# Dylan-H-Wang/skin-sm3

Measured on AMD Instinct MI355X. Metric: SM3 pretrain images/sec (paired 224x224), higher is better.
Workload: dtype bf16

## Files before the change

### include/sm3_hip.h

```cpp
#ifndef SM3_HIP_H
#define SM3_HIP_H

#include <stdint.h>

#ifdef __cplusplus
extern "C" {
#endif

#define SM3_F32 0
#define SM3_BF16 1
#define SM3_F16 2

#define SM3_EINVAL (-1)
#define SM3_EALIGN (-2)
#define SM3_EDTYPE (-3)

#define SM3_MAX_TAPS 9

int sm3_abi_version(void);

typedef struct sm3_conv_desc {
    int32_t dtype;
    int32_t N, Hi, Wi, Ci;
    int32_t Ho, Wo, Co;
    int32_t sy, sx;
    int32_t ntaps;
    int32_t dy[SM3_MAX_TAPS], dx[SM3_MAX_TAPS], wtap[SM3_MAX_TAPS];
    int32_t w_row_stride;
    int32_t Hout, Wout;
    int32_t osy, osx, ooy, oox;
} sm3_conv_desc;

int sm3_conv_partial_rows(const sm3_conv_desc* d);

int sm3_conv_gather_gemm(const sm3_conv_desc* d, const void* x, const void* w, void* y,
                         const void* addend, float* stat_partials, void* stream);

typedef struct sm3_bn_bwd_fuse {
    const uint8_t* relu_mask;
    const void* x;
    const float* mean;
    const float* invstd;
    float* partials;
    int32_t partial_row_offset;
    int32_t views;
    int32_t partial_row_offset_view1;
    int32_t addend_sp_h, addend_sp_w;
} sm3_bn_bwd_fuse;
int sm3_conv_dgrad_bnfuse(const sm3_conv_desc* d, const void* dy_in, const void* w_dgrad, void* dz_out,
                          const void* addend, const sm3_bn_bwd_fuse* fuse, void* stream);

typedef struct sm3_conv_seg {
    const void* x1;
    const void* w1;
    int32_t Ci1;
    int64_t w_view_stride;
    int64_t w1_view_stride;
    const float* col_bias;
    int32_t views;
} sm3_conv_seg;
int sm3_conv_dgrad_seg_bnfuse(const sm3_conv_desc* d, const void* x0, const void* w0, const sm3_conv_seg* seg,
                              void* dz_out, const void* addend, const sm3_bn_bwd_fuse* fuse, void* stream);
int sm3_conv_gather_gemm_seg(const sm3_conv_desc* d, const void* x0, const void* w0, const sm3_conv_seg* seg, void* y,
                             const void* addend, void* stream);
int sm3_conv_seg_act(const sm3_conv_desc* d, const void* x0, const void* w0, const sm3_conv_seg* seg, int relu, void* y,
                     uint8_t* relu_mask, void* stream);

int sm3_conv_bn_act_eval(const sm3_conv_desc* d, const void* x, const void* w, const float* scale,
                         const float* shift, const void* residual, int relu, void* y, void* stream);
int sm3_conv_bn_act_fused(const sm3_conv_desc* d, const void* x, const void* w, const float* scale, const float* shift,
                          const void* residual, int relu, void* y, uint8_t* relu_mask, int views, void* stream);
int sm3_conv_bn_eval(const sm3_conv_desc* d, const void* x, const void* w, const float* gamma, const float* beta,
                     const float* running_mean, const float* running_var, float eps, const void* residual, int relu,
                     void* y, void* stream);

int sm3_conv_wgrad(const sm3_conv_desc* d, const void* x, const void* dy, float* dw, void* stream);
int sm3_conv_wgrad_cat(const sm3_conv_desc* d, const void* x, const void* dy, float* dw, const void* dy1, int Co1,
                       float* dw1, int views, int64_t dw_view_stride, int64_t dw1_view_stride, void* stream);
int sm3_conv_wgrad_slabs(const sm3_conv_desc* d, const void* x, const void* dy, float* slabs, int slab_capacity, int views,
                         int* slabs_used, void* stream);
int sm3_slab_reduce(const float* slabs, int nslabs, int64_t n, float* out, int accumulate, void* stream);
int sm3_conv_wgrad_det(const sm3_conv_desc* d, const void* x, const void* dy, float* dw, float* slabs, int slab_capacity,
                       void* stream);

#define SM3_BN_REDUCE_GROUPS 64
int sm3_bn_reduce_groups(int rows);
int sm3_bn_stats_reduce(const float* partials, int rows, int C, double* sums, double* workspace, int views,
                        void* stream);
int sm3_bn_finalize(const double* sums, int groups , int views,
                    double count , int C, const float* gamma, const float* beta,
                    float eps, float momentum, float* running_mean, float* running_var,
                    int64_t* num_batches_tracked , float* scale, float* shift, float* save_mean,
                    float* save_invstd , void* stream);
int sm3_bn_eval_scale_shift(const float* gamma, const float* beta, const float* running_mean,
                            const float* running_var, float eps, int C, float* scale, float* shift,
                            void* stream);
int sm3_bn_act(int dtype, const void* x, const float* scale, const float* shift, const void* residual,
               int relu, int out_f32, void* y, uint8_t* relu_mask, int64_t rows, int C, int views, void* stream);
int sm3_bn_act_colsum_rows(int64_t rows, int C, int dtype);
int sm3_bn_act_colsum(int dtype, const void* x, const float* scale, const float* shift, const void* residual, int relu,
                      void* y, uint8_t* relu_mask, float* colsum_partials, int64_t rows, int C, int views, void* stream);
int sm3_subsample_colsum_rows(int64_t rows, int C, int dtype);
int sm3_subsample_colsum(int dtype, const void* x, void* y, float* colsum_partials, int N, int H, int W, int C, int stride,
                         int views, void* stream);
int sm3_bn_add_bn_act(int dtype, const void* x, const float* scale, const float* shift, const void* x2,
                      const float* scale2, const float* shift2, int relu, void* y, uint8_t* relu_mask,
                      int64_t rows, int C, int views, void* stream);
int sm3_bn_bwd_partial_rows(int64_t rows, int C);
int sm3_bn_bwd_reduce(int dtype, const void* dy, const void* y, const uint8_t* relu_mask, const void* x,
                      const float* mean, const float* invstd, void* dz, int64_t rows, int C,
                      float* partials , int views, void* stream);
int sm3_bn_bwd_apply(int dtype, const void* dz, const void* x, const float* mean, const float* invstd,
                     const float* gamma, const double* global_sums, double count,
                     const double* local_sums, float* dgamma, float* dbeta, void* dx, int64_t rows,
                     int C, int views, void* stream);

typedef struct sm3_bn_apply_side {
    const void* x;
    const float* mean;
    const float* invstd;
    const float* gamma;
    const double* global_sums;
    const double* local_sums;
    float* dgamma;
    float* dbeta;
    void* dx;
} sm3_bn_apply_side;
int sm3_bn_bwd_apply2(int dtype, const void* dz, double count, const sm3_bn_apply_side* a,
                      const sm3_bn_apply_side* b, int64_t rows, int C, int views, void* stream);

int sm3_linbn_moments(const float* slabs, int nslabs, int64_t n, float* out, const float* colsum_partials, int colsum_rows,
                      double* s_out, int p, int views, void* stream);
int sm3_linbn_fwd_stats(int dtype, const float* G, const void* w_dgrad, const void* w_fwd, const double* s, float* Tm,
                        double* sums_ws, int C, int p, int views, void* stream);
int sm3_linbn_stats(int dtype, const float* P, const void* w_fwd, const float* mean, const float* invstd, const float* gamma,
                    const double* reduce_ws, int groups, double* lsums, float* dgamma, float* dbeta, double count,
                    float* coef, int C, int p, int views, void* stream);
int sm3_linbn_coef(const double* global_sums, double count, const float* gamma, const float* mean, const float* invstd,
                   float* coef, int C, int views, void* stream);
int sm3_linbn_banks(int dtype, const void* w_dgrad, const float* coef, void* wa, void* wbn, float* col_const, int C, int p,
                    int views, void* stream);
int sm3_linbn_fold(const double* sums_ws, int groups, int n, int views, double* out, void* stream);
int sm3_linbn_scale_banks(int dtype, const void* w3, int K3, const float* scale3, const float* shift3, void* out3,
                          const void* wd, int Kd, const float* scaled, const float* shiftd, void* outd, float* bias, int C,
                          int views, void* stream);
int sm3_linbn_post(int dtype, const void* wbn, const void* w_dgrad, void* hn, const float* P, const float* G,
                   const float* Tm, const double* s, const float* coef, float* dw, int C, int p, int views, void* stream);
int sm3_linbn_banks_post(int dtype, const void* w_dgrad, const float* coef, void* wa, float* col_const, void* hn,
                         const float* P, const float* G, const float* Tm, const double* s, float* dw, int C, int p, int views,
                         void* stream);

int sm3_stem_partial_rows(int N, int H, int W);
int sm3_stem_weight_prep(int dtype, const float* w_master, void* w_stem, void* stream);
int sm3_stem_weight_prep_if(int dtype, const float* w_master, void* w_stem, const int* only_if, void* stream);
int sm3_stem_conv_fwd(int dtype, const float* x_nchw, const void* w_stem, void* y, float* stat_partials, int N, int H,
                      int W, void* stream);
#define SM3_STEM_WGRAD_SLABS 768
int sm3_stem_wgrad_bn(int dtype, const float* x_nchw, const void* dz, const void* xo, const float* mean,
                      const float* invstd, const float* gamma, const double* global_sums, double count,
                      const double* local_sums, float* dgamma, float* dbeta, float* dw, float* dw_slabs, int N, int H, int W,
                      int views, void* stream);
int sm3_stem_image_cols(int W);
int sm3_stem_image_prep(int dtype, const float* x_view0, const float* x_view1, void* ximg, int n_per_view, int views, int H,
                        int W, void* stream);
int sm3_stem_conv_fwd16(int dtype, const void* ximg, const void* w_stem, void* y, float* stat_partials, int N, int H, int W,
                        void* stream);
int sm3_stem_wgrad_bn16(int dtype, const void* ximg, const void* dz, const void* xo, const float* mean, const float* invstd,
                        const float* gamma, const double* global_sums, double count, const double* local_sums,
                        float* dgamma, float* dbeta, float* dw, float* dw_slabs, int N, int H, int W, int views,
                        void* stream);
int sm3_stem_dgrad_bn(int dtype, const void* dz, const void* xo, const float* mean, const float* invstd, const float* gamma,
                      const double* global_sums, double count, const float* w_master, float* dx, int N, int H, int W,
                      int views, void* stream);
int sm3_maxpool3x3s2_fwd(int dtype, const void* x, void* y, uint8_t* argmax, int N, int H, int W, int C, void* stream);
int sm3_maxpool3x3s2_bwd(int dtype, const uint8_t* argmax, const void* dy, void* dx, int N, int H, int W, int C,
                         void* stream);
int sm3_bn_relu_maxpool_fwd(int dtype, const void* x, const float* scale, const float* shift, void* y,
                            uint8_t* argmax, int N, int H, int W, int C, int views, void* stream);
int sm3_maxpool_bn_bwd_partial_rows(int N, int H, int W, int views);
int sm3_maxpool_bn_bwd(int dtype, const uint8_t* argmax, const void* dy, const void* x, const float* scale,
                       const float* shift, const float* mean, const float* invstd, void* dz, float* partials,
                       int N, int H, int W, int C, int views, void* stream);
int sm3_avgpool_fwd(int dtype, const void* x, float* feat_f32, void* feat_t, int N, int HW, int C, void* stream);
int sm3_avgpool_bwd(int dtype, const void* dfeat, void* dx, int N, int HW, int C, void* stream);

int sm3_weight_prep(int dtype, const float* w, int Co, int taps, int Ci, void* w_fwd, int ld_fwd,
                    void* w_dgrad, void* stream);
typedef struct sm3_wprep_item {
    const float* w;
    void* w_fwd;
    void* w_dgrad;
    int32_t Co, taps, Ci, ld_fwd;
} sm3_wprep_item;
int sm3_weight_prep_batch(int dtype, const sm3_wprep_item* items_device, int n, void* stream);
int sm3_weights_changed(const float* flat, int64_t n, uint64_t* state, int* changed, void* stream);
int sm3_weight_prep_batch_if(int dtype, const sm3_wprep_item* items_device, int n, const int* only_if, void* stream);
int sm3_cast_from_f32(int dtype, const float* src, void* dst, int64_t n, void* stream);
int sm3_cast_to_f32(int dtype, const void* src, float* dst, int64_t n, void* stream);

int sm3_ntxent_logits(const float* z, int R, int D, float temperature, float* zn, float* inv_norm,
                      float* logits, void* stream);
int sm3_ntxent_logits_bwd(int dtype, const float* dlogits, const float* zn, const float* inv_norm, int R,
                          int D, float temperature, void* dz, void* stream);
int sm3_ce_label0(const float* logits, int R, int Cc, float weight, float* row_terms, float* loss, float* dlogits,
                  void* stream);
int sm3_ntxent_fused(int dtype, const float* z, int R, int D, float temperature, float weight,
                     float* workspace, float* loss, void* dz, void* stream);

int sm3_ntxent_fused_scaled(int dtype, const float* z, int R, int D, float temperature, float weight,
                            const float* dz_scale, float* workspace, float* loss, void* dz, void* stream);

int sm3_ntxent_fused_batch(int dtype, int nterms, const float* const* z, int R, int D, float temperature, const float* weights,
                           const float* dz_scale, float* workspace, float* loss, void* const* dz, void* stream);

int sm3_normalize_rows(const float* z, int R, int D, float* zn, float* inv_norm, void* stream);
int sm3_ntxent_rect(float* S, int Rl, int Rg, int self_offset, float temperature, float weight, const float* dz_scale,
                    float* row_terms , float* loss, void* stream);
int sm3_normalize_rows_bwd(int dtype, const float* dzn_a, const float* dzn_b, const float* zn, const float* inv_norm,
                           int R, int D, void* dz, void* stream);

int sm3_adamw(float* p, const float* g, float* m, float* v, int64_t n, float lr, float beta1, float beta2,
              float eps, float weight_decay, int step, float grad_scale, const int32_t* found_inf,
              void* stream);
int sm3_adamw_dynamic(float* p, const float* g, float* m, float* v, int64_t n, float lr, float beta1, float beta2,
                      float eps, float weight_decay, float grad_scale, const float* loss_scale,
                      const int32_t* steps_taken, const int32_t* found_inf, void* stream);
int sm3_loss_scale_update(float* loss_scale, int32_t* found_inf, int32_t* growth_tracker, int32_t* steps_taken,
                          float growth_factor, float backoff_factor, int growth_interval, void* stream);
int sm3_ema_update(float* target, const float* online, int64_t n, float momentum, void* stream);
int sm3_check_finite(const float* g, int64_t n, int32_t* found_inf, void* stream);

int sm3_aug_resized_crop(const uint8_t* src, int B, int Hs, int Ws, const int32_t* box, const uint8_t* flip, float* out,
                         int H, int W, void* stream);
int sm3_aug_resized_crop_ragged(const uint8_t* arena, int64_t arena_bytes, const int64_t* offset, const int32_t* img_h,
                                const int32_t* img_w, int n_images, const int32_t* index, const int32_t* box,
                                const uint8_t* flip, int B, float* out, int H, int W, void* stream);
int sm3_aug_color_op(float* img, int B, int H, int W, const int32_t* op, const float* factor, float* gray_mean, void* stream);
int sm3_aug_finish(const float* img, int B, int H, int W, const uint8_t* gray, const float* sigma, const float* mean3,
                   const float* std3, float* out, void* stream);

int sm3_token_attention(int dtype, const void* qkv, void* out, int B, int S, int D, int nhead, void* stream);
int sm3_add_layernorm(int dtype, const void* a, const void* b, const float* gamma, const float* beta, float eps,
                      void* out, int64_t rows, int D, void* stream);
int sm3_token_heads(int dtype, const void* x, const float* W, const float* bias, const int* token_of, int l2_norm,
                    float* out, int B, int S, int D, int T, void* stream);

int sm3_mlc_attention_fwd(const float* qkv, float* out, int B, int S, int D, int nhead, float p, uint32_t seed,
                          int label_major, void* stream);
int sm3_mlc_attention_bwd(const float* qkv, const float* dout, float* dqkv, int B, int S, int D, int nhead, float p,
                          uint32_t seed, int label_major, void* stream);
int sm3_mlc_add_ln_fwd(const float* a, const float* b, const float* gamma, const float* beta, float eps, float p,
                       uint32_t seed, float* out, float* stats, int64_t rows, int D, void* stream);
int sm3_mlc_add_ln_bwd(const float* dout, const float* a, const float* b, const float* stats, const float* gamma, float p,
                       uint32_t seed, float* da, float* db, float* dgamma, float* dbeta, int64_t rows, int D, void* stream);
int sm3_mlc_bias_relu_drop_fwd(const float* y, const float* bias, float p, uint32_t seed, float* h, float* hd, int64_t rows,
                               int N, void* stream);
int sm3_mlc_relu_drop_bwd(const float* dhd, const float* h, float p, uint32_t seed, float* dh, float* dbias, int64_t rows,
                          int N, void* stream);
int sm3_mlc_colsum(const float* dy, float* db, int64_t rows, int N, void* stream);
int sm3_mlc_ce(const float* logits, const int64_t* targets, const int* head_offsets, int H, int B, int Tn, float temperature,
               float* loss, float* dlogits, void* stream);
int sm3_mlc_heads_fwd(const float* x, const float* W, const float* bias, const int* token_of, int l2_norm, float* out, int B,
                      int S, int D, int Tn, int label_major, void* stream);
int sm3_mlc_heads_bwd(const float* dlogits, const float* x, const float* W, const int* token_of, int l2_norm, float* dx,
                      float* dW, float* dbias, int B, int S, int D, int Tn, int label_major, void* stream);
int sm3_mlc_kmeans_assign(const float* emb, const float* centroids, int64_t* assign, float* sums, int* counts, int N, int D,
                          int K, void* stream);
int sm3_mlc_kmeans_update(float* centroids, const float* sums, const int* counts, int K, int D, void* stream);

#define SM3_MLC_SLAB_ROWS 256
int sm3_mlc_colsum_det(const float* dy, float* db, float* slabs, int64_t rows, int N, int groups, void* stream);
int sm3_mlc_add_ln_bwd_det(const float* dout, const float* a, const float* b, const float* stats, const float* gamma, float p,
                           uint32_t seed, float* da, float* db, float* dgamma, float* dbeta, float* slabs, int64_t rows, int D,
                           void* stream);
int sm3_mlc_heads_bwd_det(const float* dlogits, const float* x, const float* W, const int* token_of, int l2_norm, float* dx,
                          float* dW, float* dbias, float* work, int B, int S, int D, int Tn, int label_major, void* stream);
int sm3_mlc_kmeans_assign_det(const float* emb, const float* centroids, int64_t* assign, float* sums, int* counts, float* slabs,
                              int N, int D, int K, void* stream);

int sm3_grouped_gemm(int dtype, const void* x, const void* w, void* y, float* stat_partials, int rows, int groups, int K, int N,
                     void* stream);
int sm3_grouped_wgrad_det(int dtype, const void* x, const void* dy, float* dw, float* slabs, int slab_capacity, int rows,
                          int groups, int K, int N, void* stream);

int sm3_gconv_weight_prep(int dtype, const float* master, void* w_fwd, void* w_dgrad, int C, int groups, const int* only_if,
                          void* stream);
int sm3_gconv_fwd(int dtype, const void* x, const void* w_fwd, void* y, float* stat_partials, int N, int H, int W, int C,
                  int groups, int stride, void* stream);
int sm3_gconv_dgrad(int dtype, const void* dy, const void* w_dgrad, void* dx, int N, int H, int W, int C, int groups, int stride,
                    void* stream);
int sm3_gconv_wgrad_slabs(int N, int H, int W, int stride, int slab_capacity);
int sm3_gconv_wgrad_det(int dtype, const void* x, const void* dy, float* dw, float* slabs, int slab_capacity, int N, int H,
                        int W, int C, int groups, int stride, void* stream);

int sm3_p2p_mailbox_bytes(void);
int sm3_p2p_max_elems(void);
int sm3_p2p_max_world(void);
int sm3_p2p_layout(int slot, int src, int block, int64_t* data_first, int64_t* data_bytes, int64_t* flag_off,
                   int* elems_per_block);
int sm3_p2p_alloc(void** ptr, void* ipc_handle_64, int* kind_out);
int sm3_p2p_open(const void* ipc_handle_64, void** ptr);
int sm3_p2p_close(void* ptr);
int sm3_p2p_free(void* ptr);
int sm3_p2p_allreduce_f64(double* buf, int n, void* const* mailboxes, int rank, int world, uint64_t seq, int* err_flag,
                          double timeout_s, void* stream);

int sm3_knn_vote(const float* S, int64_t B, int64_t N, int64_t ld, const int32_t* targets, int L, const int32_t* class_offsets,
                 int k, float temperature, float* scores, int32_t* nbr_idx, float* nbr_sim, void* stream);

int sm3_cam_alpha(int dtype, const void* g, float* alpha, int T, int N, int HW, int C, void* stream);
int sm3_cam_maps(int dtype, const void* a, const float* alpha, float* low, float* maps, int N, int T, int h, int w, int C, int H,
                 int W, void* stream);

int sm3_attr_path(const float* x, const float* base, int base_n, float* out, int N, int64_t E, int k0, int c, int steps,
                  void* stream);
int sm3_attr_noise(const float* x, const float* sigma, float* out, int N, int64_t E, int k0, int c, int stride, uint64_t seed,
                   void* stream);
int sm3_attr_accumulate(const float* g, float* acc, int c, int N, int64_t E, float weight, int squared, void* stream);
int sm3_attr_finish_blocks(int HW);
int sm3_attr_finish(const float* acc, const float* x, const float* base, int base_n, float* attr, float* maps, double* sums,
                    double* partials, int T, int N, int C, int HW, int mode, void* stream);

int sm3_faith_rank_workspace(int rows, int HW);
// ... 16 lines not shown
```

### skin-sm3_amd/csrc/pool.hip

```cpp
#include "common.h"

namespace {

template <typename T>
__device__ __forceinline__ void store_elem(T* p, float v);
template <>
__device__ __forceinline__ void store_elem<float>(float* p, float v) { *p = v; }
template <>
__device__ __forceinline__ void store_elem<bf16_t>(bf16_t* p, float v) { p->v = f32_to_bf16(v); }
template <>
__device__ __forceinline__ void store_elem<f16_t>(f16_t* p, float v) { p->v = f32_to_f16(v); }

struct PixDiv {
    FastDiv cv, w, hw;
};
static PixDiv make_pixdiv(int cv, int w, int h) {
    PixDiv d;
    d.cv = make_fastdiv((uint32_t)cv);
    d.w = make_fastdiv((uint32_t)w);
    d.hw = make_fastdiv((uint32_t)(w * h));
    return d;
}
__device__ __forceinline__ void split_index(uint32_t idx, const PixDiv& d, int& c, uint32_t& pix, int& n, int& y, int& x) {
    pix = fdiv(idx, d.cv);
    c = (int)(idx - pix * d.cv.d);
    n = (int)fdiv(pix, d.hw);
    const uint32_t rem = pix - (uint32_t)n * d.hw.d;
    y = (int)fdiv(rem, d.w);
    x = (int)(rem - (uint32_t)y * d.w.d);
}

template <typename T>
__global__ __launch_bounds__(256) void maxpool_fwd_kernel(const T* __restrict__ x, T* __restrict__ y,
                                                          uint8_t* __restrict__ argmax, int N, int H, int W, int C,
                                                          int Ho, int Wo, uint32_t total, const PixDiv dv) {
    constexpr int E = ElemTraits<T>::kPer16B;
    for (uint32_t idx = blockIdx.x * blockDim.x + threadIdx.x; idx < total; idx += gridDim.x * blockDim.x) {
        int c, n, oy, ox;
        uint32_t pix32;
        split_index(idx, dv, c, pix32, n, oy, ox);
        const int64_t pix = pix32;
        float best[E];
        int arg[E];
#pragma unroll
        for (int e = 0; e < E; ++e) {
            best[e] = -INFINITY;
            arg[e] = -1;
        }
#pragma unroll
        for (int kh = 0; kh < 3; ++kh) {
            const int iy = oy * 2 - 1 + kh;
            if ((unsigned)iy >= (unsigned)H) continue;
#pragma unroll
            for (int kw = 0; kw < 3; ++kw) {
                const int ix = ox * 2 - 1 + kw;
                if ((unsigned)ix >= (unsigned)W) continue;
                float v[E];
                unpack16<T>(*reinterpret_cast<const uint4*>(x + (((int64_t)n * H + iy) * W + ix) * C + (int64_t)c * E), v);
#pragma unroll
                for (int e = 0; e < E; ++e)
                    if (v[e] > best[e] || arg[e] < 0) {
                        best[e] = v[e];
                        arg[e] = kh * 3 + kw;
                    }
            }
        }
        *reinterpret_cast<uint4*>(y + pix * C + (int64_t)c * E) = pack16<T>(best);
        if (argmax) {
            uint8_t* a = argmax + pix * C + (int64_t)c * E;
            if constexpr (E == 8) {
                *reinterpret_cast<uint2*>(a) = make_uint2(
                    (unsigned)arg[0] | ((unsigned)arg[1] << 8) | ((unsigned)arg[2] << 16) | ((unsigned)arg[3] << 24),
                    (unsigned)arg[4] | ((unsigned)arg[5] << 8) | ((unsigned)arg[6] << 16) | ((unsigned)arg[7] << 24));
            } else {
                *reinterpret_cast<unsigned*>(a) =
                    (unsigned)arg[0] | ((unsigned)arg[1] << 8) | ((unsigned)arg[2] << 16) | ((unsigned)arg[3] << 24);
            }
        }
    }
}

template <typename T>
__global__ __launch_bounds__(256) void maxpool_bwd_kernel(const uint8_t* __restrict__ argmax, const T* __restrict__ dy,
                                                          T* __restrict__ dx, int N, int H, int W, int C, int Ho,
                                                          int Wo, uint32_t total, const PixDiv dv) {
    constexpr int E = ElemTraits<T>::kPer16B;
    for (uint32_t idx = blockIdx.x * blockDim.x + threadIdx.x; idx < total; idx += gridDim.x * blockDim.x) {
        int c, n, iy, ix;
        uint32_t pix32;
        split_index(idx, dv, c, pix32, n, iy, ix);
        const int64_t pix = pix32;
        float g[E];
#pragma unroll
        for (int e = 0; e < E; ++e) g[e] = 0.f;
        const int oy_lo = iy / 2, oy_hi = min(Ho - 1, (iy + 1) / 2);
        const int ox_lo = ix / 2, ox_hi = min(Wo - 1, (ix + 1) / 2);
        for (int oy = oy_lo; oy <= oy_hi; ++oy)
            for (int ox = ox_lo; ox <= ox_hi; ++ox) {
                const int self = (iy - (oy * 2 - 1)) * 3 + (ix - (ox * 2 - 1));
                const int64_t o = (((int64_t)n * Ho + oy) * Wo + ox) * C + (int64_t)c * E;
                unsigned a[2];
                if constexpr (E == 8) {
                    const uint2 q = *reinterpret_cast<const uint2*>(argmax + o);
                    a[0] = q.x;
                    a[1] = q.y;
                } else {
                    a[0] = *reinterpret_cast<const unsigned*>(argmax + o);
                    a[1] = 0;
                }
                float d[E];
                unpack16<T>(*reinterpret_cast<const uint4*>(dy + o), d);
#pragma unroll
                for (int e = 0; e < E; ++e)
                    if ((int)((a[e >> 2] >> (8 * (e & 3))) & 0xff) == self) g[e] += d[e];
            }
        *reinterpret_cast<uint4*>(dx + pix * C + (int64_t)c * E) = pack16<T>(g);
    }
}

template <typename T>
__global__ __launch_bounds__(256) void bn_relu_maxpool_fwd_kernel(const T* __restrict__ x, const float* __restrict__ scale,
                                                                  const float* __restrict__ shift, T* __restrict__ y,
                                                                  uint8_t* __restrict__ argmax, int N, int H, int W, int C,
                                                                  int Ho, int Wo, int n_per_view, uint32_t total,
                                                                  const PixDiv dv) {
    constexpr int E = ElemTraits<T>::kPer16B;
    for (uint32_t idx = blockIdx.x * blockDim.x + threadIdx.x; idx < total; idx += gridDim.x * blockDim.x) {
        int c, n, oy, ox;
        uint32_t pix32;
        split_index(idx, dv, c, pix32, n, oy, ox);
        const int64_t pix = pix32;
        const int view = n / n_per_view;
        float sc[E], sh[E], best[E];
        int arg[E];
#pragma unroll
        for (int e = 0; e < E; ++e) {
            sc[e] = scale[view * C + c * E + e];
            sh[e] = shift[view * C + c * E + e];
            best[e] = -INFINITY;
            arg[e] = -1;
        }
#pragma unroll
        for (int kh = 0; kh < 3; ++kh) {
            const int iy = oy * 2 - 1 + kh;
            if ((unsigned)iy >= (unsigned)H) continue;
#pragma unroll
            for (int kw = 0; kw < 3; ++kw) {
                const int ix = ox * 2 - 1 + kw;
                if ((unsigned)ix >= (unsigned)W) continue;
                float v[E];
                unpack16<T>(*reinterpret_cast<const uint4*>(x + (((int64_t)n * H + iy) * W + ix) * C + (int64_t)c * E), v);
#pragma unroll
                for (int e = 0; e < E; ++e) {
                    const float a = ElemTraits<T>::round(fmaxf(v[e] * sc[e] + sh[e], 0.f));
                    if (a > best[e] || arg[e] < 0) {
                        best[e] = a;
                        arg[e] = kh * 3 + kw;
                    }
                }
            }
        }
        *reinterpret_cast<uint4*>(y + pix * C + (int64_t)c * E) = pack16<T>(best);
        if (argmax) {
            uint8_t* a = argmax + pix * C + (int64_t)c * E;
            if constexpr (E == 8) {
                *reinterpret_cast<uint2*>(a) = make_uint2(
                    (unsigned)arg[0] | ((unsigned)arg[1] << 8) | ((unsigned)arg[2] << 16) | ((unsigned)arg[3] << 24),
                    (unsigned)arg[4] | ((unsigned)arg[5] << 8) | ((unsigned)arg[6] << 16) | ((unsigned)arg[7] << 24));
            } else {
                *reinterpret_cast<unsigned*>(a) =
                    (unsigned)arg[0] | ((unsigned)arg[1] << 8) | ((unsigned)arg[2] << 16) | ((unsigned)arg[3] << 24);
            }
        }
    }
}

template <typename T>
__global__ __launch_bounds__(256) void maxpool_bn_bwd_kernel(const uint8_t* __restrict__ argmax, const T* __restrict__ dy,
                                                             const T* __restrict__ x, const float* __restrict__ scale,
                                                             const float* __restrict__ shift,
                                                             const float* __restrict__ mean,
                                                             const float* __restrict__ invstd, T* __restrict__ dz,
                                                             float* __restrict__ partials, int H, int W, int C, int Ho,
                                                             int Wo, int n_per_view, int64_t rows, int tbx, int tby,
                                                             const FastDiv div_hw, const FastDiv div_w) {
    constexpr int E = ElemTraits<T>::kPer16B;
    __shared__ float sred[256 * 2 * 8];
    const int tx = threadIdx.x % tbx, ty = threadIdx.x / tbx;
    const int cv = blockIdx.x * tbx + tx;
    const bool active = (cv * E < C) && (ty < tby);
    const int view = blockIdx.z;
    float s1[E], s2[E];
#pragma unroll
    for (int e = 0; e < E; ++e) s1[e] = s2[e] = 0.f;
    if (active) {
        float sc[E], sh[E], mu[E], is[E];
#pragma unroll
        for (int e = 0; e < E; ++e) {
            sc[e] = scale[view * C + cv * E + e];
            sh[e] = shift[view * C + cv * E + e];
            mu[e] = mean[view * C + cv * E + e];
            is[e] = invstd[view * C + cv * E + e];
        }
        constexpr int U = 2;
        const int64_t rstep = (int64_t)gridDim.y * tby;
        for (int64_t r0 = (int64_t)blockIdx.y * tby + ty; r0 < rows; r0 += U * rstep) {
            uint4 xu[U], du[U][4];
            unsigned au[U][4][2];
            int selfs[U][4];
            int64_t pixs[U];
#pragma unroll
            for (int u = 0; u < U; ++u) {
                const int64_t r = r0 + u * rstep;
                pixs[u] = -1;
                xu[u] = make_uint4(0, 0, 0, 0);
#pragma unroll
                for (int w = 0; w < 4; ++w) selfs[u][w] = -1;
                if (r >= rows) continue;
                const uint32_t nl = fdiv((uint32_t)r, div_hw);
                const uint32_t rem = (uint32_t)r - nl * div_hw.d;
                const int iy = (int)fdiv(rem, div_w), ix = (int)(rem - (uint32_t)iy * div_w.d);
                const int64_t n = (int64_t)view * n_per_view + nl;
                pixs[u] = (int64_t)view * rows + r;
                xu[u] = ldg16<true>(x + pixs[u] * C + (int64_t)cv * E);
                const int oy_lo = iy / 2, oy_hi = min(Ho - 1, (iy + 1) / 2);
                const int ox_lo = ix / 2, ox_hi = min(Wo - 1, (ix + 1) / 2);
#pragma unroll
                for (int w = 0; w < 4; ++w) {
                    const int oy = oy_lo + (w >> 1), ox = ox_lo + (w & 1);
                    if (oy > oy_hi || ox > ox_hi) continue;
                    selfs[u][w] = (iy - (oy * 2 - 1)) * 3 + (ix - (ox * 2 - 1));
                    const int64_t o = ((n * Ho + oy) * Wo + ox) * C + (int64_t)cv * E;
                    if constexpr (E == 8) {
                        const uint2 q = *reinterpret_cast<const uint2*>(argmax + o);
                        au[u][w][0] = q.x;
                        au[u][w][1] = q.y;
                    } else {
                        au[u][w][0] = *reinterpret_cast<const unsigned*>(argmax + o);
                        au[u][w][1] = 0;
                    }
                    du[u][w] = *reinterpret_cast<const uint4*>(dy + o);
                }
            }
#pragma unroll
            for (int u = 0; u < U; ++u) {
                if (pixs[u] < 0) continue;
                float g[E];
#pragma unroll
                for (int e = 0; e < E; ++e) g[e] = 0.f;
#pragma unroll
                for (int w = 0; w < 4; ++w) {
                    if (selfs[u][w] < 0) continue;
                    float d[E];
                    unpack16<T>(du[u][w], d);
#pragma unroll
                    for (int e = 0; e < E; ++e)
                        if ((int)((au[u][w][e >> 2] >> (8 * (e & 3))) & 0xff) == selfs[u][w]) g[e] += d[e];
                }
                float xv[E];
                unpack16<T>(xu[u], xv);
#pragma unroll
                for (int e = 0; e < E; ++e) g[e] = (xv[e] * sc[e] + sh[e] > ElemTraits<T>::kReluBit) ? g[e] : 0.f;
                const uint4 packed = pack16<T>(g);
                stg16<true>(dz + pixs[u] * C + (int64_t)cv * E, packed);
                float gr[E];
                unpack16<T>(packed, gr);
#pragma unroll
                for (int e = 0; e < E; ++e) {
                    s1[e] += gr[e];
                    s2[e] += gr[e] * (xv[e] - mu[e]) * is[e];
                }
            }
        }
    }
    float* mine = sred + threadIdx.x * 2 * E;
#pragma unroll
    for (int e = 0; e < E; ++e) {
        mine[e] = s1[e];
        mine[E + e] = s2[e];
    }
    __syncthreads();
    if (ty == 0 && cv * E < C) {
        for (int j = 1; j < tby; ++j) {
            const float* o = sred + (j * tbx + tx) * 2 * E;
#pragma unroll
            for (int e = 0; e < E; ++e) {
                s1[e] += o[e];
                s2[e] += o[E + e];
            }
        }
        float* pv = partials + (int64_t)view * gridDim.y * 2 * C;
        float* p1 = pv + ((int64_t)blockIdx.y * 2 + 0) * C + (int64_t)cv * E;
        float* p2 = pv + ((int64_t)blockIdx.y * 2 + 1) * C + (int64_t)cv * E;
#pragma unroll
        for (int e = 0; e < E; ++e) {
            p1[e] = s1[e];
            p2[e] = s2[e];
        }
    }
}

template <typename T>
__global__ __launch_bounds__(256) void avgpool_fwd_kernel(const T* __restrict__ x, float* __restrict__ f32,
                                                          T* __restrict__ ft, int N, int HW, int C) {
    constexpr int E = ElemTraits<T>::kPer16B;
    const int cv = C / E;
    const int64_t total = (int64_t)N * cv;
    const int64_t idx = (int64_t)blockIdx.x * blockDim.x + threadIdx.x;
    if (idx >= total) return;
    const int c = (int)(idx % cv);
    const int n = (int)(idx / cv);
    float s[E];
#pragma unroll
    for (int e = 0; e < E; ++e) s[e] = 0.f;
    for (int i = 0; i < HW; ++i) {
        float v[E];
        unpack16<T>(*reinterpret_cast<const uint4*>(x + ((int64_t)n * HW + i) * C + (int64_t)c * E), v);
#pragma unroll
        for (int e = 0; e < E; ++e) s[e] += v[e];
    }
    const float inv = 1.f / (float)HW;
#pragma unroll
    for (int e = 0; e < E; ++e) s[e] *= inv;
    if (f32) {
#pragma unroll
        for (int e = 0; e < E; ++e) f32[(int64_t)n * C + (int64_t)c * E + e] = s[e];
    }
    if (ft) *reinterpret_cast<uint4*>(ft + (int64_t)n * C + (int64_t)c * E) = pack16<T>(s);
}

template <typename T>
__global__ __launch_bounds__(256) void avgpool_bwd_kernel(const T* __restrict__ df, T* __restrict__ dx, int N, int HW,
                                                          int C) {
    constexpr int E = ElemTraits<T>::kPer16B;
    const int cv = C / E;
    const int64_t total = (int64_t)N * HW * cv;
    const float inv = 1.f / (float)HW;
    for (int64_t idx = (int64_t)blockIdx.x * blockDim.x + threadIdx.x; idx < total;
         idx += (int64_t)gridDim.x * blockDim.x) {
        const int c = (int)(idx % cv);
        const int64_t pix = idx / cv;
        const int n = (int)(pix / HW);
        float v[E];
        unpack16<T>(*reinterpret_cast<const uint4*>(df + (int64_t)n * C + (int64_t)c * E), v);
#pragma unroll
        for (int e = 0; e < E; ++e) v[e] *= inv;
        *reinterpret_cast<uint4*>(dx + pix * C + (int64_t)c * E) = pack16<T>(v);
    }
}

template <typename T>
__global__ void weight_prep_kernel(const float* __restrict__ w, int Co, int taps, int Ci, T* __restrict__ wf, int ld,
                                   T* __restrict__ wd) {
    const int64_t nf = wf ? (int64_t)Co * ld : 0;
    const int64_t nd = wd ? (int64_t)Co * taps * Ci : 0;
    const int K = taps * Ci;
    for (int64_t idx = (int64_t)blockIdx.x * blockDim.x + threadIdx.x; idx < nf + nd;
         idx += (int64_t)gridDim.x * blockDim.x) {
        if (idx < nf) {
            const int co = (int)(idx / ld), k = (int)(idx % ld);
            store_elem<T>(wf + idx, k < K ? w[(int64_t)co * K + k] : 0.f);
        } else {
            const int64_t j = idx - nf;
            const int co = (int)(j % Co);
            const int t = (int)((j / Co) % taps);
            const int ci = (int)(j / ((int64_t)Co * taps));
            store_elem<T>(wd + j, w[((int64_t)co * taps + t) * Ci + ci]);
        }
    }
}

template <typename T>
__global__ __launch_bounds__(256) void weight_prep_batch_kernel(const sm3_wprep_item* __restrict__ items,
                                                                const int* __restrict__ only_if) {
    __shared__ float tile[32][33];
    if (only_if && *only_if == 0) return;
    const sm3_wprep_item it = items[blockIdx.y];
    const float* __restrict__ w = it.w;
    T* __restrict__ wf = reinterpret_cast<T*>(it.w_fwd);
    T* __restrict__ wd = reinterpret_cast<T*>(it.w_dgrad);
    const int Co = it.Co, taps = it.taps, Ci = it.Ci, ld = it.ld_fwd, K = taps * Ci;
    const bool vec = sizeof(T) == 2 && ld == K && (K & 3) == 0 && (Co & 1) == 0 && ((uintptr_t)w & 15) == 0 &&
                     ((uintptr_t)wf & 7) == 0 && ((uintptr_t)wd & 3) == 0;
    if (wf && vec) {
        const int64_t nq = (int64_t)Co * K / 4;
        const float4* __restrict__ w4 = reinterpret_cast<const float4*>(w);
        uint2* __restrict__ o2 = reinterpret_cast<uint2*>(wf);
        for (int64_t q = (int64_t)blockIdx.x * blockDim.x + threadIdx.x; q < nq; q += (int64_t)gridDim.x * blockDim.x) {
            const float4 v = w4[q];
            uint2 o;
            if constexpr (sizeof(T) == 2) {
                o.x = pack2<T>(v.x, v.y);
                o.y = pack2<T>(v.z, v.w);
            }
            o2[q] = o;
        }
    } else if (wf) {
        const int64_t nf = (int64_t)Co * ld;
        for (int64_t idx = (int64_t)blockIdx.x * blockDim.x + threadIdx.x; idx < nf; idx += (int64_t)gridDim.x * blockDim.x) {
            const int co = (int)(idx / ld), k = (int)(idx % ld);
            store_elem<T>(wf + idx, k < K ? w[(int64_t)co * K + k] : 0.f);
        }
    }
    if (wd && vec) {
        __shared__ float tile2[64][33];
        const int tco = (Co + 63) / 64, tci = (Ci + 31) / 32;
        const int ntiles = taps * tco * tci;
        const int tx = threadIdx.x & 31, ty = threadIdx.x >> 5;
        for (int tl = blockIdx.x; tl < ntiles; tl += gridDim.x) {
            const int t = tl / (tco * tci), r = tl - t * tco * tci;
            const int co0 = (r / tci) * 64, ci0 = (r % tci) * 32;
#pragma unroll
            for (int j = 0; j < 8; ++j) {
                const int co = co0 + ty + 8 * j, ci = ci0 + tx;
                tile2[ty + 8 * j][tx] = (co < Co && ci < Ci) ? w[((int64_t)co * taps + t) * Ci + ci] : 0.f;
            }
            __syncthreads();
#pragma unroll
            for (int j = 0; j < 4; ++j) {
                const int ci = ci0 + ty + 8 * j, co = co0 + 2 * tx;
                if constexpr (sizeof(T) == 2) {
                    if (ci < Ci && co < Co)
                        *reinterpret_cast<uint32_t*>(wd + ((int64_t)ci * taps + t) * Co + co) =
                            pack2<T>(tile2[2 * tx][ty + 8 * j], tile2[2 * tx + 1][ty + 8 * j]);
                }
            }
            __syncthreads();
        }
    } else if (wd) {
        const int tco = (Co + 31) / 32, tci = (Ci + 31) / 32;
        const int ntiles = taps * tco * tci;
        const int tx = threadIdx.x & 31, ty = threadIdx.x >> 5;
        for (int tl = blockIdx.x; tl < ntiles; tl += gridDim.x) {
            const int t = tl / (tco * tci), r = tl - t * tco * tci;
            const int co0 = (r / tci) * 32, ci0 = (r % tci) * 32;
#pragma unroll
            for (int j = 0; j < 4; ++j) {
                const int co = co0 + ty + 8 * j, ci = ci0 + tx;
                tile[ty + 8 * j][tx] = (co < Co && ci < Ci) ? w[((int64_t)co * taps + t) * Ci + ci] : 0.f;
            }
            __syncthreads();
#pragma unroll
            for (int j = 0; j < 4; ++j) {
                const int ci = ci0 + ty + 8 * j, co = co0 + tx;
                if (ci < Ci && co < Co) store_elem<T>(wd + ((int64_t)ci * taps + t) * Co + co, tile[tx][ty + 8 * j]);
            }
            __syncthreads();
        }
    }
}

template <typename T>
__global__ void cast_from_f32_kernel(const float* __restrict__ s, T* __restrict__ d, int64_t n) {
    for (int64_t i = (int64_t)blockIdx.x * blockDim.x + threadIdx.x; i < n; i += (int64_t)gridDim.x * blockDim.x)
        store_elem<T>(d + i, s[i]);
}
template <typename T>
__global__ void cast_to_f32_kernel(const T* __restrict__ s, float* __restrict__ d, int64_t n) {
    for (int64_t i = (int64_t)blockIdx.x * blockDim.x + threadIdx.x; i < n; i += (int64_t)gridDim.x * blockDim.x)
        d[i] = ElemTraits<T>::load(s + i);
}

inline unsigned grid_for(int64_t total, int per_block = 256, int64_t cap = 8192) {
    int64_t g = (total + per_block - 1) / per_block;
    if (g > cap) g = cap;
    if (g < 1) g = 1;
    return (unsigned)g;
}

}

#define DISPATCH_T(dtype, CALL_F32, CALL_BF16, CALL_F16)  \
    if ((dtype) == SM3_F32) { CALL_F32; }       \
    else if ((dtype) == SM3_BF16) { CALL_BF16; } \
    else if ((dtype) == SM3_F16) { CALL_F16; } \
    else return SM3_EDTYPE;

extern "C" int sm3_maxpool3x3s2_fwd(int dtype, const void* x, void* y, uint8_t* argmax, int N, int H, int W, int C,
                                    void* stream) {
    if (!x || !y || N <= 0 || H <= 0 || W <= 0 || C <= 0) return SM3_EINVAL;
    const int E = dtype == SM3_F32 ? 4 : 8;
    if (C % E) return SM3_EALIGN;
    const int Ho = (H + 2 - 3) / 2 + 1, Wo = (W + 2 - 3) / 2 + 1;
    const int64_t total = (int64_t)N * Ho * Wo * (C / E);
    if (total >= 0x7fffffffLL) return SM3_EINVAL;
    const unsigned g = grid_for(total, 256, 1 << 20);
    hipStream_t st = (hipStream_t)stream;
    const PixDiv dv = make_pixdiv(C / E, Wo, Ho);
    DISPATCH_T(dtype,
               hipLaunchKernelGGL(maxpool_fwd_kernel<float>, dim3(g), dim3(256), 0, st, (const float*)x, (float*)y, argmax, N, H, W, C, Ho, Wo, (uint32_t)total, dv),
               hipLaunchKernelGGL(maxpool_fwd_kernel<bf16_t>, dim3(g), dim3(256), 0, st, (const bf16_t*)x, (bf16_t*)y, argmax, N, H, W, C, Ho, Wo, (uint32_t)total, dv),
               hipLaunchKernelGGL(maxpool_fwd_kernel<f16_t>, dim3(g), dim3(256), 0, st, (const f16_t*)x, (f16_t*)y, argmax, N, H, W, C, Ho, Wo, (uint32_t)total, dv));
    SM3_CHECK_LAUNCH();
    return 0;
}

extern "C" int sm3_maxpool3x3s2_bwd(int dtype, const uint8_t* argmax, const void* dy, void* dx, int N, int H, int W,
                                    int C, void* stream) {
    if (!argmax || !dy || !dx || N <= 0 || H <= 0 || W <= 0 || C <= 0) return SM3_EINVAL;
    const int E = dtype == SM3_F32 ? 4 : 8;
    if (C % E) return SM3_EALIGN;
    const int Ho = (H + 2 - 3) / 2 + 1, Wo = (W + 2 - 3) / 2 + 1;
    const int64_t total = (int64_t)N * H * W * (C / E);
    if (total >= 0x7fffffffLL) return SM3_EINVAL;
    const unsigned g = grid_for(total, 256, 1 << 20);
    hipStream_t st = (hipStream_t)stream;
    const PixDiv dv = make_pixdiv(C / E, W, H);
    DISPATCH_T(dtype,
               hipLaunchKernelGGL(maxpool_bwd_kernel<float>, dim3(g), dim3(256), 0, st, argmax, (const float*)dy, (float*)dx, N, H, W, C, Ho, Wo, (uint32_t)total, dv),
               hipLaunchKernelGGL(maxpool_bwd_kernel<bf16_t>, dim3(g), dim3(256), 0, st, argmax, (const bf16_t*)dy, (bf16_t*)dx, N, H, W, C, Ho, Wo, (uint32_t)total, dv),
               hipLaunchKernelGGL(maxpool_bwd_kernel<f16_t>, dim3(g), dim3(256), 0, st, argmax, (const f16_t*)dy, (f16_t*)dx, N, H, W, C, Ho, Wo, (uint32_t)total, dv));
    SM3_CHECK_LAUNCH();
    return 0;
}

extern "C" int sm3_bn_relu_maxpool_fwd(int dtype, const void* x, const float* scale, const float* shift, void* y,
                                       uint8_t* argmax, int N, int H, int W, int C, int views, void* stream) {
    if (!x || !scale || !shift || !y || N <= 0 || H <= 0 || W <= 0 || C <= 0 || views < 1 || N % views) return SM3_EINVAL;
    if (!SM3_DTYPE_OK(dtype)) return SM3_EDTYPE;
    const int E = dtype == SM3_F32 ? 4 : 8;
    if (C % E) return SM3_EALIGN;
    const int Ho = (H + 2 - 3) / 2 + 1, Wo = (W + 2 - 3) / 2 + 1;
    const int64_t total = (int64_t)N * Ho * Wo * (C / E);
    if (total >= 0x7fffffffLL) return SM3_EINVAL;
    const unsigned g = grid_for(total, 256, 1 << 20);
    hipStream_t st = (hipStream_t)stream;
    const PixDiv dv = make_pixdiv(C / E, Wo, Ho);
    DISPATCH_T(dtype,
               hipLaunchKernelGGL(bn_relu_maxpool_fwd_kernel<float>, dim3(g), dim3(256), 0, st, (const float*)x, scale, shift, (float*)y, argmax, N, H, W, C, Ho, Wo, N / views, (uint32_t)total, dv),
               hipLaunchKernelGGL(bn_relu_maxpool_fwd_kernel<bf16_t>, dim3(g), dim3(256), 0, st, (const bf16_t*)x, scale, shift, (bf16_t*)y, argmax, N, H, W, C, Ho, Wo, N / views, (uint32_t)total, dv),
               hipLaunchKernelGGL(bn_relu_maxpool_fwd_kernel<f16_t>, dim3(g), dim3(256), 0, st, (const f16_t*)x, scale, shift, (f16_t*)y, argmax, N, H, W, C, Ho, Wo, N / views, (uint32_t)total, dv));
    SM3_CHECK_LAUNCH();
    return 0;
}

extern "C" int sm3_maxpool_bn_bwd_partial_rows(int N, int H, int W, int views) {
    if (N <= 0 || H <= 0 || W <= 0 || views < 1 || N % views) return SM3_EINVAL;
    int64_t gy = ((int64_t)(N / views) * H * W + 63) / 64;
    return (int)(gy > 1024 ? 1024 : gy);
}

extern "C" int sm3_maxpool_bn_bwd(int dtype, const uint8_t* argmax, const void* dy, const void* x, const float* scale,
                                  const float* shift, const float* mean, const float* invstd, void* dz,
                                  float* partials, int N, int H, int W, int C, int views, void* stream) {
    if (!argmax || !dy || !x || !scale || !shift || !mean || !invstd || !dz || !partials) return SM3_EINVAL;
    if (N <= 0 || H <= 0 || W <= 0 || C <= 0 || views < 1 || N % views) return SM3_EINVAL;
    if (!SM3_DTYPE_OK(dtype)) return SM3_EDTYPE;
    const int E = dtype == SM3_F32 ? 4 : 8;
    if (C % E || C / E > 256) return SM3_EALIGN;
    const int Ho = (H + 2 - 3) / 2 + 1, Wo = (W + 2 - 3) / 2 + 1;
    const int64_t rows = (int64_t)(N / views) * H * W;
    if (rows * views >= 0x7fffffffLL) return SM3_EINVAL;
    const int cvecs = C / E;
    int tbx = 1;
    while (tbx < cvecs && tbx < 256) tbx <<= 1;
    const int tby = 256 / tbx;
    const int gx = (cvecs + tbx - 1) / tbx;
    const int gy = sm3_maxpool_bn_bwd_partial_rows(N, H, W, views);
    hipStream_t st = (hipStream_t)stream;
    const FastDiv dhw = make_fastdiv((uint32_t)(H * W)), dw = make_fastdiv((uint32_t)W);
    dim3 grid(gx, gy, views);
    DISPATCH_T(dtype,
               hipLaunchKernelGGL(maxpool_bn_bwd_kernel<float>, grid, dim3(256), 0, st, argmax, (const float*)dy, (const float*)x, scale, shift, mean, invstd, (float*)dz, partials, H, W, C, Ho, Wo, N / views, rows, tbx, tby, dhw, dw),
               hipLaunchKernelGGL(maxpool_bn_bwd_kernel<bf16_t>, grid, dim3(256), 0, st, argmax, (const bf16_t*)dy, (const bf16_t*)x, scale, shift, mean, invstd, (bf16_t*)dz, partials, H, W, C, Ho, Wo, N / views, rows, tbx, tby, dhw, dw),
               hipLaunchKernelGGL(maxpool_bn_bwd_kernel<f16_t>, grid, dim3(256), 0, st, argmax, (const f16_t*)dy, (const f16_t*)x, scale, shift, mean, invstd, (f16_t*)dz, partials, H, W, C, Ho, Wo, N / views, rows, tbx, tby, dhw, dw));
    SM3_CHECK_LAUNCH();
    return 0;
}

extern "C" int sm3_avgpool_fwd(int dtype, const void* x, float* feat_f32, void* feat_t, int N, int HW, int C,
                               void* stream) {
    if (!x || N <= 0 || HW <= 0 || C <= 0 || (!feat_f32 && !feat_t)) return SM3_EINVAL;
    const int E = dtype == SM3_F32 ? 4 : 8;
    if (C % E) return SM3_EALIGN;
    const int64_t total = (int64_t)N * (C / E);
    const unsigned g = (unsigned)((total + 255) / 256);
    hipStream_t st = (hipStream_t)stream;
    DISPATCH_T(dtype,
               hipLaunchKernelGGL(avgpool_fwd_kernel<float>, dim3(g), dim3(256), 0, st, (const float*)x, feat_f32, (float*)feat_t, N, HW, C),
               hipLaunchKernelGGL(avgpool_fwd_kernel<bf16_t>, dim3(g), dim3(256), 0, st, (const bf16_t*)x, feat_f32, (bf16_t*)feat_t, N, HW, C),
               hipLaunchKernelGGL(avgpool_fwd_kernel<f16_t>, dim3(g), dim3(256), 0, st, (const f16_t*)x, feat_f32, (f16_t*)feat_t, N, HW, C));
    SM3_CHECK_LAUNCH();
    return 0;
}

extern "C" int sm3_avgpool_bwd(int dtype, const void* dfeat, void* dx, int N, int HW, int C, void* stream) {
    if (!dfeat || !dx || N <= 0 || HW <= 0 || C <= 0) return SM3_EINVAL;
    const int E = dtype == SM3_F32 ? 4 : 8;
    if (C % E) return SM3_EALIGN;
    const unsigned g = grid_for((int64_t)N * HW * (C / E));
    hipStream_t st = (hipStream_t)stream;
    DISPATCH_T(dtype,
               hipLaunchKernelGGL(avgpool_bwd_kernel<float>, dim3(g), dim3(256), 0, st, (const float*)dfeat, (float*)dx, N, HW, C),
               hipLaunchKernelGGL(avgpool_bwd_kernel<bf16_t>, dim3(g), dim3(256), 0, st, (const bf16_t*)dfeat, (bf16_t*)dx, N, HW, C),
               hipLaunchKernelGGL(avgpool_bwd_kernel<f16_t>, dim3(g), dim3(256), 0, st, (const f16_t*)dfeat, (f16_t*)dx, N, HW, C));
    SM3_CHECK_LAUNCH();
    return 0;
}

extern "C" int sm3_weight_prep(int dtype, const float* w, int Co, int taps, int Ci, void* w_fwd, int ld_fwd,
                               void* w_dgrad, void* stream) {
    if (!w || Co <= 0 || taps <= 0 || Ci <= 0 || (!w_fwd && !w_dgrad)) return SM3_EINVAL;
    if (w_fwd && ld_fwd < taps * Ci) return SM3_EINVAL;
    const int64_t total = (w_fwd ? (int64_t)Co * ld_fwd : 0) + (w_dgrad ? (int64_t)Co * taps * Ci : 0);
    const unsigned g = grid_for(total);
    hipStream_t st = (hipStream_t)stream;
    DISPATCH_T(dtype,
               hipLaunchKernelGGL(weight_prep_kernel<float>, dim3(g), dim3(256), 0, st, w, Co, taps, Ci, (float*)w_fwd, ld_fwd, (float*)w_dgrad),
               hipLaunchKernelGGL(weight_prep_kernel<bf16_t>, dim3(g), dim3(256), 0, st, w, Co, taps, Ci, (bf16_t*)w_fwd, ld_fwd, (bf16_t*)w_dgrad),
               hipLaunchKernelGGL(weight_prep_kernel<f16_t>, dim3(g), dim3(256), 0, st, w, Co, taps, Ci, (f16_t*)w_fwd, ld_fwd, (f16_t*)w_dgrad));
    SM3_CHECK_LAUNCH();
    return 0;
}

extern "C" int sm3_weight_prep_batch_if(int dtype, const sm3_wprep_item* items_device, int n, const int* only_if,
                                        void* stream) {
    if (!items_device || n <= 0 || n > 65535) return SM3_EINVAL;
    static const int kWprepGx = getenv("SM3_WPREP_GX") ? atoi(getenv("SM3_WPREP_GX")) : 384;
    hipStream_t st = (hipStream_t)stream;
    DISPATCH_T(dtype,
               hipLaunchKernelGGL(weight_prep_batch_kernel<float>, dim3(kWprepGx, n), dim3(256), 0, st, items_device, only_if),
               hipLaunchKernelGGL(weight_prep_batch_kernel<bf16_t>, dim3(kWprepGx, n), dim3(256), 0, st, items_device, only_if),
               hipLaunchKernelGGL(weight_prep_batch_kernel<f16_t>, dim3(kWprepGx, n), dim3(256), 0, st, items_device, only_if));
    SM3_CHECK_LAUNCH();
    return 0;
}

extern "C" int sm3_weight_prep_batch(int dtype, const sm3_wprep_item* items_device, int n, void* stream) {
    return sm3_weight_prep_batch_if(dtype, items_device, n, nullptr, stream);
}

namespace {

__global__ __launch_bounds__(256) void weights_hash_kernel(const uint32_t* __restrict__ w, int64_t n,
                                                           unsigned long long* __restrict__ acc) {
    unsigned long long h = 0;
    const int64_t stride = (int64_t)gridDim.x * blockDim.x;
    for (int64_t i = (int64_t)blockIdx.x * blockDim.x + threadIdx.x; i < n; i += stride)
        h += ((unsigned long long)w[i] + 0x9E3779B97F4A7C15ull) * (unsigned long long)(2 * i + 1);
#pragma unroll
    for (int o = 32; o > 0; o >>= 1) h += __shfl_xor(h, o, 64);
    __shared__ unsigned long long part[4];
    if ((threadIdx.x & 63) == 0) part[threadIdx.x >> 6] = h;
    __syncthreads();
    if (threadIdx.x == 0) atomicAdd(acc, part[0] + part[1] + part[2] + part[3]);
}

__global__ void weights_changed_kernel(unsigned long long* __restrict__ state, int* __restrict__ changed) {
    *changed = state[0] != state[1];
    state[1] = state[0];
    state[0] = 0;
}

}

extern "C" int sm3_weights_changed(const float* flat, int64_t n, uint64_t* state, int* changed, void* stream) {
    if (!flat || !state || !changed || n <= 0) return SM3_EINVAL;
    hipStream_t st = (hipStream_t)stream;
    hipLaunchKernelGGL(weights_hash_kernel, dim3(1024), dim3(256), 0, st, reinterpret_cast<const uint32_t*>(flat), n,
                       reinterpret_cast<unsigned long long*>(state));
    SM3_CHECK_LAUNCH();
    hipLaunchKernelGGL(weights_changed_kernel, dim3(1), dim3(1), 0, st, reinterpret_cast<unsigned long long*>(state), changed);
    SM3_CHECK_LAUNCH();
    return 0;
}

extern "C" int sm3_cast_from_f32(int dtype, const float* src, void* dst, int64_t n, void* stream) {
    if (!src || !dst || n <= 0) return SM3_EINVAL;
    const unsigned g = grid_for(n);
    hipStream_t st = (hipStream_t)stream;
    DISPATCH_T(dtype,
               hipLaunchKernelGGL(cast_from_f32_kernel<float>, dim3(g), dim3(256), 0, st, src, (float*)dst, n),
               hipLaunchKernelGGL(cast_from_f32_kernel<bf16_t>, dim3(g), dim3(256), 0, st, src, (bf16_t*)dst, n),
               hipLaunchKernelGGL(cast_from_f32_kernel<f16_t>, dim3(g), dim3(256), 0, st, src, (f16_t*)dst, n));
    SM3_CHECK_LAUNCH();
    return 0;
}

extern "C" int sm3_cast_to_f32(int dtype, const void* src, float* dst, int64_t n, void* stream) {
    if (!src || !dst || n <= 0) return SM3_EINVAL;
    const unsigned g = grid_for(n);
    hipStream_t st = (hipStream_t)stream;
    DISPATCH_T(dtype,
               hipLaunchKernelGGL(cast_to_f32_kernel<float>, dim3(g), dim3(256), 0, st, (const float*)src, dst, n),
               hipLaunchKernelGGL(cast_to_f32_kernel<bf16_t>, dim3(g), dim3(256), 0, st, (const bf16_t*)src, dst, n),
               hipLaunchKernelGGL(cast_to_f32_kernel<f16_t>, dim3(g), dim3(256), 0, st, (const f16_t*)src, dst, n));
    SM3_CHECK_LAUNCH();
    return 0;
}
```

### skin-sm3_amd/csrc/stem.hip

```cpp
#include <atomic>

#include "conv_common.h"

namespace {

constexpr int PW = 264;
constexpr int NG = 21;
constexpr int KS = 11;
constexpr int KPAD = KS * 16;
constexpr int OUT_PITCH = 144;

struct StemTile {
    int n, oy, x0;
};
__device__ __forceinline__ StemTile decode_tile(long t, int xblocks, int Ho) {
    StemTile s;
    const int xb = (int)(t % xblocks);
    const long r = t / xblocks;
    s.oy = (int)(r % Ho);
    s.n = (int)(r / Ho);
    s.x0 = xb * 128;
    return s;
}

// ... 277 lines not shown
constexpr int PATCH16 = PDMA * 1024;

template <typename T>
__global__ __launch_bounds__(256) void stem_image_prep_kernel(const float* __restrict__ x0, const float* __restrict__ x1,
                                                              uint4* __restrict__ out, int n_per_view, int H, int W, int Wp8,
                                                              long chunks) {
    const long i = (long)blockIdx.x * 256 + threadIdx.x;
    if (i >= chunks) return;
    const int j = (int)(i % Wp8);
    const long r = i / Wp8;
    const long rows_img = 3L * H;
    const int n = (int)(r / rows_img);
    const long rr = r - (long)n * rows_img;
    const float* src = (n < n_per_view ? x0 + (long)n * rows_img * W : x1 + (long)(n - n_per_view) * rows_img * W) + rr * W;
    float v[8];
    const int q0 = 8 * j - 4;
    if ((W & 3) == 0 && q0 >= 0 && q0 + 8 < W && (((uintptr_t)src) & 15) == 0) {
        const float4 a = *reinterpret_cast<const float4*>(src + q0), b = *reinterpret_cast<const float4*>(src + q0 + 4);
        v[0] = a.y; v[1] = a.z; v[2] = a.w; v[3] = b.x; v[4] = b.y; v[5] = b.z; v[6] = b.w; v[7] = src[q0 + 8];
    } else {
#pragma unroll
        for (int e = 0; e < 8; ++e) {
            const int q = 8 * j + e - 3;
            v[e] = (unsigned)q < (unsigned)W ? src[q] : 0.f;
        }
    }
    out[i] = make_uint4(pack2<T>(v[0], v[1]), pack2<T>(v[2], v[3]), pack2<T>(v[4], v[5]), pack2<T>(v[6], v[7]));
}

struct TileDiv {
    FastDiv xb, ho;
};
__device__ __forceinline__ StemTile decode_tile32(uint32_t t, const TileDiv& d) {
    StemTile s;
    const uint32_t r = fdiv(t, d.xb), xb = t - r * d.xb.d;
    const uint32_t n = fdiv(r, d.ho);
    s.oy = (int)(r - n * d.ho.d);
    s.n = (int)n;
    s.x0 = (int)xb * 128;
    return s;
}

__device__ __forceinline__ void patch_dma(__amdgpu_buffer_rsrc_t rs, uint32_t lds_patch, const StemTile& t, int H, int Wp,
                                          int wave, int lane) {
    for (int k = wave; k < PDMA; k += 4) {
        const int idx = k * 64 + lane;
        const int g = idx / PCH, j = idx - g * PCH;
        const int kh = g / 3, c = g - 3 * kh;
        const int iy = 2 * t.oy - 3 + kh, q = 2 * t.x0 + 8 * j;
        const bool ok = g < NG && (unsigned)iy < (unsigned)H && q < Wp;
        const uint32_t off = ok ? (uint32_t)((((long)t.n * 3 + c) * H + iy) * Wp + q) * 2u : sm3conv::kOOB;
        sm3conv::dma16(rs, lds_patch + (uint32_t)k * 1024u, off, 0u);
    }
}

constexpr int FWD16_LDS = 2 * PATCH16 + 128 * OUT_PITCH + 4 * 64 * 2 * 4 + 64 * (KPAD + 8) * 2;

template <typename T>
__global__ __launch_bounds__(256, 2) void stem_fwd16_kernel(const char* __restrict__ ximg, uint32_t ximg_bytes,
                                                          const uint4* __restrict__ w, T* __restrict__ y,
                                                          float* __restrict__ partials, int H, int Wp, int Ho, int Wo,
                                                          const TileDiv td, uint32_t tiles) {
    extern __shared__ __attribute__((aligned(16))) char smem16[];
    char* sPatch = smem16;
    char* sOut = smem16 + 2 * PATCH16;
    float(*sStat)[64][2] = reinterpret_cast<float(*)[64][2]>(sOut + 128 * OUT_PITCH);
    constexpr int WP = KPAD + 8;
    uint16_t* sW = reinterpret_cast<uint16_t*>(sOut + 128 * OUT_PITCH + 4 * 64 * 2 * 4);
    const int tid = threadIdx.x, lane = tid & 63, wave = __builtin_amdgcn_readfirstlane(tid >> 6);
    const int col = lane & 31, h = lane >> 5;
    for (int i = tid; i < 64 * (KPAD / 8); i += 256) {
        const int co = i / (KPAD / 8), c8 = i - co * (KPAD / 8);
        *reinterpret_cast<uint4*>(&sW[co * WP + c8 * 8]) = w[i];
    }
    const uint16_t* wlane = &sW[col * WP + 8 * h];
    const __amdgpu_buffer_rsrc_t rs = __builtin_amdgcn_make_buffer_rsrc((void*)ximg, 0, ximg_bytes, 0x00020000);
    const uint32_t lds_patch = (uint32_t)(uintptr_t)((__attribute__((address_space(3))) char*)sPatch);

    int buf = 0;
    if (blockIdx.x < tiles) patch_dma(rs, lds_patch, decode_tile32(blockIdx.x, td), H, Wp, wave, lane);
    sm3conv::dma_drain();
    for (uint32_t t = blockIdx.x; t < tiles; t += gridDim.x, buf ^= 1) {
        const StemTile tl = decode_tile32(t, td);
        const uint32_t tn = t + gridDim.x;
        __syncthreads();
        if (tn < tiles)
            patch_dma(rs, lds_patch + (uint32_t)((buf ^ 1) * PATCH16), decode_tile32(tn, td), H, Wp, wave, lane);
        f32x16 acc[2];
#pragma unroll
        for (int nb = 0; nb < 2; ++nb)
#pragma unroll
            for (int r = 0; r < 16; ++r) acc[nb][r] = 0.f;
        const int px = 32 * wave + col;
        const char* prow = sPatch + buf * PATCH16 + 4 * px;
#pragma unroll
        for (int ks = 0; ks < KS; ++ks) {
            const int g = 2 * ks + h;
            uint4 a = make_uint4(0, 0, 0, 0);
            if (g < NG) {
                const uint32_t* src = reinterpret_cast<const uint32_t*>(prow + g * PROW16);
                a = make_uint4(src[0], src[1], src[2], src[3]);
            }
#pragma unroll
            for (int nb = 0; nb < 2; ++nb)
                sm3conv::mma_frag<T>(a, *reinterpret_cast<const uint4*>(wlane + nb * 32 * WP + ks * 16), acc[nb]);
        }
#pragma unroll
        for (int nb = 0; nb < 2; ++nb) {
            float s1 = 0.f, s2 = 0.f;
#pragma unroll
            for (int r = 0; r < 16; ++r) {
                const int row = 32 * wave + (r & 3) + 8 * (r >> 2) + 4 * h;
                const uint16_t b = (uint16_t)pack2<T>(acc[nb][r], 0.f);
                *reinterpret_cast<uint16_t*>(sOut + row * OUT_PITCH + (nb * 32 + col) * 2) = b;
                if (tl.x0 + row < Wo) {
                    const float v = ElemTraits<T>::round(acc[nb][r]);
                    s1 += v;
                    s2 += v * v;
                }
            }
            s1 += __shfl_xor(s1, 32, 64);
            s2 += __shfl_xor(s2, 32, 64);
            if (lane < 32) {
                sStat[wave][nb * 32 + lane][0] = s1;
                sStat[wave][nb * 32 + lane][1] = s2;
            }
        }
        sm3conv::dma_drain();
        __syncthreads();
        if (partials && tid < 128) {
            const int c = tid & 63, st = tid >> 6;
            partials[((long)t * 2 + st) * 64 + c] = (sStat[0][c][st] + sStat[1][c][st]) + (sStat[2][c][st] + sStat[3][c][st]);
        }
        {
            const int ch = tid & 7, r0 = tid >> 3;
            const long pix0 = ((long)tl.n * Ho + tl.oy) * Wo + tl.x0;
#pragma unroll
            for (int k = 0; k < 4; ++k) {
                const int row = r0 + 32 * k;
                if (tl.x0 + row < Wo)
                    stg16<true>(y + (pix0 + row) * 64 + ch * 8,
                                *reinterpret_cast<const uint4*>(sOut + row * OUT_PITCH + ch * 16));
            }
        }
    }
}

struct StemWgrad16Params {
    StemWgradParams q;
    const char* ximg;
    uint32_t ximg_bytes;
    int Wp;
    TileDiv td;
};

template <typename T>
__global__ __launch_bounds__(256, 3) void stem_wgrad16_kernel(const StemWgrad16Params pp) {
    const StemWgradParams& p = pp.q;
    __shared__ __attribute__((aligned(16))) char sPatch[2 * PATCH16];
    __shared__ __attribute__((aligned(16))) char sD[128 * 128];
    __shared__ __attribute__((aligned(16))) float sCoef[3][64];
    const int tid = threadIdx.x, lane = tid & 63, wave = __builtin_amdgcn_readfirstlane(tid >> 6);
    const int cb = wave & 1, kb0 = 3 * (wave >> 1);

    if (blockIdx.x == 0 && tid < 64 && p.lsums) {
        float db = 0.f, dg = 0.f;
        for (int v = 0; v < p.views; ++v) {
            db += (float)p.lsums[v * 128 + tid];
            dg += (float)p.lsums[v * 128 + 64 + tid];
        }
        if (p.dbeta) atomicAdd(&p.dbeta[tid], db);
        if (p.dgamma) atomicAdd(&p.dgamma[tid], dg);
    }

    f32x16 acc[3];
#pragma unroll
    for (int j = 0; j < 3; ++j)
#pragma unroll
        for (int r = 0; r < 16; ++r) acc[j][r] = 0.f;

    const int ch = tid & 7, r0 = tid >> 3;
    int cur_view = -1;
    const int g16 = lane >> 4, ii = lane & 15, qq = ii >> 2, pq = ii & 3, hh = g16 >> 1;
    const uint32_t ra_off = (uint32_t)(8 * hh + qq) * 128u + ((((uint32_t)(cb * 32 + 16 * (g16 & 1) + 4 * pq)) * 2u) ^ swz128(qq));
    const int bn = lane & 31, bh = lane >> 5;
    const __amdgpu_buffer_rsrc_t rs = __builtin_amdgcn_make_buffer_rsrc((void*)pp.ximg, 0, pp.ximg_bytes, 0x00020000);
    const uint32_t lds_patch = (uint32_t)(uintptr_t)((__attribute__((address_space(3))) char*)sPatch);
    uint32_t b_off[3], b_sel[3];
#pragma unroll
    for (int j = 0; j < 3; ++j) {
        const int k = 32 * (kb0 + j) + bn, g = k >> 3, kw = k & 7;
        b_off[j] = g < NG ? (uint32_t)(g * PROW16 + 4 * (8 * bh + (kw >> 1))) : 0xffffffffu;
        b_sel[j] = (kw & 1) ? 0x07060302u : 0x05040100u;
    }

    auto stage_dxo = [&](const StemTile& tl) {
        const int view = tl.n / p.n_per_view;
        if (view != cur_view) {
            cur_view = view;
            if (tid < 64) {
                const int c = tid;
                const float is = p.invstd[view * 64 + c];
                const float g = p.gamma ? p.gamma[c] : 1.f;
                const float k0c = g * is;
                const float k1c = (float)(p.gsums[view * 128 + c] * p.inv_count);
                const float qc = k0c * is * (float)(p.gsums[view * 128 + 64 + c] * p.inv_count);
                sCoef[0][c] = k0c;
                sCoef[1][c] = qc;
                sCoef[2][c] = qc * p.mean[view * 64 + c] - k0c * k1c;
            }
            __syncthreads();
        }
        float cA[8], cB[8], cC[8];
#pragma unroll
        for (int e = 0; e < 8; e += 4) {
            *reinterpret_cast<float4*>(cA + e) = *reinterpret_cast<const float4*>(&sCoef[0][ch * 8 + e]);
            *reinterpret_cast<float4*>(cB + e) = *reinterpret_cast<const float4*>(&sCoef[1][ch * 8 + e]);
            *reinterpret_cast<float4*>(cC + e) = *reinterpret_cast<const float4*>(&sCoef[2][ch * 8 + e]);
        }
        const long pix0 = ((long)tl.n * p.Ho + tl.oy) * p.Wo + tl.x0;
#pragma unroll
        for (int kb = 0; kb < 4; kb += 2) {
            uint4 gu[2], xu[2];
#pragma unroll
            for (int k = 0; k < 2; ++k) {
                const int row = r0 + 32 * (kb + k);
                const bool ok = tl.x0 + row < p.Wo;
                gu[k] = ok ? ldg16<true>(p.dz + ((pix0 + row) * 64 + ch * 8) * 2) : make_uint4(0, 0, 0, 0);
                xu[k] = ok ? ldg16<true>(p.xo + ((pix0 + row) * 64 + ch * 8) * 2) : make_uint4(0, 0, 0, 0);
            }
#pragma unroll
            for (int k = 0; k < 2; ++k) {
                const int row = r0 + 32 * (kb + k);
                uint4 out = make_uint4(0, 0, 0, 0);
                if (tl.x0 + row < p.Wo) {
                    float g[8], xv[8];
                    unpack16<T>(gu[k], g);
                    unpack16<T>(xu[k], xv);
#pragma unroll
                    for (int e = 0; e < 8; ++e) g[e] = cA[e] * g[e] - cB[e] * xv[e] + cC[e];
                    out = pack16<T>(g);
                }
                *reinterpret_cast<uint4*>(sD + row * 128 + (((uint32_t)ch * 16u) ^ swz128(row))) = out;
            }
        }
    };

    int buf = 0;
    const uint32_t ntiles = (uint32_t)p.tiles;
    if (blockIdx.x < ntiles) {
        const StemTile t0 = decode_tile32(blockIdx.x, pp.td);
        patch_dma(rs, lds_patch, t0, p.H, pp.Wp, wave, lane);
        stage_dxo(t0);
    }
    sm3conv::dma_drain();
    for (uint32_t t = blockIdx.x; t < ntiles; t += gridDim.x, buf ^= 1) {
        const uint32_t tn = t + gridDim.x;
        __syncthreads();
        StemTile nx = {0, 0, 0};
        if (tn < ntiles) {
            nx = decode_tile32(tn, pp.td);
            patch_dma(rs, lds_patch + (uint32_t)((buf ^ 1) * PATCH16), nx, p.H, pp.Wp, wave, lane);
        }
        const char* patch = sPatch + buf * PATCH16;
#pragma unroll
        for (int s = 0; s < 8; ++s) {
            const char* a0 = sD + ra_off + s * 16 * 128;
            const s16x4 lo = __builtin_amdgcn_ds_read_tr16_b64_v4i16((__attribute__((address_space(3))) s16x4*)(a0));
            const s16x4 hi = __builtin_amdgcn_ds_read_tr16_b64_v4i16((__attribute__((address_space(3))) s16x4*)(a0 + 4 * 128));
            const uint2 l2 = __builtin_bit_cast(uint2, lo), h2 = __builtin_bit_cast(uint2, hi);
            const uint4 fa = make_uint4(l2.x, l2.y, h2.x, h2.y);
#pragma unroll
            for (int j = 0; j < 3; ++j) {
                uint4 fb = make_uint4(0, 0, 0, 0);
                if (b_off[j] != 0xffffffffu) {
                    const uint32_t* d = reinterpret_cast<const uint32_t*>(patch + b_off[j] + s * 64);
                    fb = make_uint4(__builtin_amdgcn_perm(d[1], d[0], b_sel[j]), __builtin_amdgcn_perm(d[3], d[2], b_sel[j]),
                                    __builtin_amdgcn_perm(d[5], d[4], b_sel[j]), __builtin_amdgcn_perm(d[7], d[6], b_sel[j]));
                }
                sm3conv::mma_frag<T>(fa, fb, acc[j]);
            }
        }
        __syncthreads();
        if (tn < ntiles) stage_dxo(nx);
        sm3conv::dma_drain();
    }

    const int frow = lane & 31, fh = lane >> 5;
#pragma unroll
    for (int j = 0; j < 3; ++j) {
        const int k = 32 * (kb0 + j) + frow;
        const int g = k >> 3, kw = k & 7;
        if (g >= NG || kw >= 7) continue;
        const int kh = g / 3, c = g - 3 * kh;
        const int kcol = (kh * 7 + kw) * 3 + c;
#pragma unroll
        for (int r = 0; r < 16; ++r) {
            const int co = cb * 32 + (r & 3) + 8 * (r >> 2) + 4 * fh;
            if (p.dw_slabs) p.dw_slabs[(long)blockIdx.x * (64 * 147) + co * 147 + kcol] = acc[j][r];
            else atomicAdd(p.dw + co * 147 + kcol, acc[j][r]);
        }
    }
}

template <typename T>
__global__ void stem_weight_prep_kernel(const float* __restrict__ w, T* __restrict__ out, const int* __restrict__ only_if) {
    const int i = blockIdx.x * blockDim.x + threadIdx.x;
    if (i >= 64 * KPAD || (only_if && *only_if == 0)) return;
    const int co = i / KPAD, k = i - co * KPAD;
    const int g = k >> 3, kw = k & 7;
    float v = 0.f;
    if (g < NG && kw < 7) {
        const int kh = g / 3, c = g - 3 * kh;
        v = w[co * 147 + (kh * 7 + kw) * 3 + c];
    }
    out[i].v = (uint16_t)pack2<T>(v, 0.f);
}


constexpr int WPF = 172;

__global__ __launch_bounds__(256, 2) void stem_fwd_f32_kernel(const float* __restrict__ x, const float* __restrict__ w,
                                                              float* __restrict__ y, float* __restrict__ partials, int N,
                                                              int H, int W, int Ho, int Wo, int xblocks, long tiles) {
    __shared__ __attribute__((aligned(16))) float patch[NG * PW];
    __shared__ float sStat[4][64][2];
    __shared__ __attribute__((aligned(16))) float sW[64 * WPF];
    const int tid = threadIdx.x, lane = tid & 63, wave = tid >> 6;
    const int col = lane & 31, h = lane >> 5;
    for (int i = tid; i < 64 * (NG * 8 / 4); i += 256) {
        const int co = i / (NG * 2), c4 = i - co * (NG * 2);
        *reinterpret_cast<float4*>(&sW[co * WPF + c4 * 4]) = *reinterpret_cast<const float4*>(w + (long)co * KPAD + c4 * 4);
    }
    const float* wlane = &sW[col * WPF + 4 * h];

    PatchRegs pre;
    if ((long)blockIdx.x < tiles) {
        load_patch(pre, x, decode_tile(blockIdx.x, xblocks, Ho), H, W);
        store_patch(patch, pre);
    }
    __syncthreads();
    for (long t = blockIdx.x; t < tiles; t += gridDim.x) {
        const StemTile tl = decode_tile(t, xblocks, Ho);
        const long tn = t + gridDim.x;
        if (tn < tiles) load_patch(pre, x, decode_tile(tn, xblocks, Ho), H, W);
        f32x16 acc[2];
#pragma unroll
        for (int nb = 0; nb < 2; ++nb)
#pragma unroll
            for (int r = 0; r < 16; ++r) acc[nb][r] = 0.f;
        const int px = 32 * wave + col;
#pragma unroll
        for (int g = 0; g < NG; ++g) {
            const float2* src = reinterpret_cast<const float2*>(patch + g * PW + 2 * px + 4 * h);
            const float2 v0 = src[0], v1 = src[1];
            const uint4 a = make_uint4(__float_as_uint(v0.x), __float_as_uint(v0.y), __float_as_uint(v1.x), __float_as_uint(v1.y));
#pragma unroll
            for (int nb = 0; nb < 2; ++nb)
                sm3conv::mma_frag<float>(a, *reinterpret_cast<const uint4*>(wlane + nb * 32 * WPF + g * 8), acc[nb]);
        }
        const long pix0 = ((long)tl.n * Ho + tl.oy) * Wo + tl.x0;
#pragma unroll
        for (int nb = 0; nb < 2; ++nb) {
            float s1 = 0.f, s2 = 0.f;
#pragma unroll
            for (int r = 0; r < 16; ++r) {
                const int row = 32 * wave + (r & 3) + 8 * (r >> 2) + 4 * h;
                if (tl.x0 + row < Wo) {
                    const float v = acc[nb][r];
                    y[(pix0 + row) * 64 + nb * 32 + col] = v;
                    s1 += v;
                    s2 += v * v;
                }
            }
            s1 += __shfl_xor(s1, 32, 64);
            s2 += __shfl_xor(s2, 32, 64);
            if (lane < 32) {
                sStat[wave][nb * 32 + lane][0] = s1;
                sStat[wave][nb * 32 + lane][1] = s2;
            }
        }
        __syncthreads();
        if (partials && tid < 128) {
            const int c = tid & 63, st = tid >> 6;
            partials[(t * 2 + st) * 64 + c] = (sStat[0][c][st] + sStat[1][c][st]) + (sStat[2][c][st] + sStat[3][c][st]);
        }
        if (tn < tiles) store_patch(patch, pre);
        __syncthreads();
    }
}

__global__ __launch_bounds__(256, 2) void stem_wgrad_f32_kernel(const StemWgradParams p) {
    __shared__ __attribute__((aligned(16))) float patch[NG * PW];
    __shared__ __attribute__((aligned(16))) float sD[128 * 64];
    __shared__ __attribute__((aligned(16))) float sCoef[3][64];
    const int tid = threadIdx.x, lane = tid & 63, wave = tid >> 6;
// ... 313 lines not shown
    tiles = (long)N * Ho * xblocks;
    if ((long)N * 3 * H * W >= 0x7fffffffL || (long)N * Ho * Wo >= 0x7fffffffL / 64) return SM3_EINVAL;
    return 0;
}

}

extern "C" int sm3_stem_partial_rows(int N, int H, int W) {
    int Ho, Wo, xb;
    long tiles;
    if (stem_geometry(N, H, W, Ho, Wo, xb, tiles)) return SM3_EINVAL;
    return tiles > 0x7fffffffL ? SM3_EINVAL : (int)tiles;
}

extern "C" int sm3_stem_weight_prep_if(int dtype, const float* w_master, void* w_stem, const int* only_if, void* stream) {
    if (!w_master || !w_stem) return SM3_EINVAL;
    if (dtype == SM3_BF16)
        hipLaunchKernelGGL(stem_weight_prep_kernel<bf16_t>, dim3((64 * KPAD + 255) / 256), dim3(256), 0, (hipStream_t)stream,
                           w_master, (bf16_t*)w_stem, only_if);
    else if (dtype == SM3_F16)
        hipLaunchKernelGGL(stem_weight_prep_kernel<f16_t>, dim3((64 * KPAD + 255) / 256), dim3(256), 0, (hipStream_t)stream,
                           w_master, (f16_t*)w_stem, only_if);
    else if (dtype == SM3_F32)
        hipLaunchKernelGGL(stem_weight_prep_f32_kernel, dim3((64 * KPAD + 255) / 256), dim3(256), 0, (hipStream_t)stream,
                           w_master, (float*)w_stem, only_if);
    else
        return SM3_EDTYPE;
    SM3_CHECK_LAUNCH();
    return 0;
}

extern "C" int sm3_stem_weight_prep(int dtype, const float* w_master, void* w_stem, void* stream) {
    return sm3_stem_weight_prep_if(dtype, w_master, w_stem, nullptr, stream);
}

extern "C" int sm3_stem_conv_fwd(int dtype, const float* x_nchw, const void* w_stem, void* y, float* stat_partials, int N,
                                 int H, int W, void* stream) {
    if (!x_nchw || !w_stem || !y) return SM3_EINVAL;
    if (dtype != SM3_BF16 && dtype != SM3_F16 && dtype != SM3_F32) return SM3_EDTYPE;
    int Ho, Wo, xb;
    long tiles;
    if (int rc = stem_geometry(N, H, W, Ho, Wo, xb, tiles)) return rc;
    if (dtype == SM3_F32) {
        const unsigned gridf = (unsigned)(tiles < 512 ? tiles : 512);
        hipLaunchKernelGGL(stem_fwd_f32_kernel, dim3(gridf), dim3(256), 0, (hipStream_t)stream, x_nchw, (const float*)w_stem,
                           (float*)y, stat_partials, N, H, W, Ho, Wo, xb, tiles);
        SM3_CHECK_LAUNCH();
        return 0;
    }
    const unsigned grid = (unsigned)(tiles < 768 ? tiles : 768);
    if (dtype == SM3_BF16)
        hipLaunchKernelGGL(stem_fwd_kernel<bf16_t>, dim3(grid), dim3(256), 0, (hipStream_t)stream, x_nchw,
                           (const uint4*)w_stem, (bf16_t*)y, stat_partials, N, H, W, Ho, Wo, xb, tiles);
    else
        hipLaunchKernelGGL(stem_fwd_kernel<f16_t>, dim3(grid), dim3(256), 0, (hipStream_t)stream, x_nchw,
                           (const uint4*)w_stem, (f16_t*)y, stat_partials, N, H, W, Ho, Wo, xb, tiles);
    SM3_CHECK_LAUNCH();
    return 0;
}

extern "C" int sm3_stem_wgrad_bn(int dtype, const float* x_nchw, const void* dz, const void* xo, const float* mean,
                                 const float* invstd, const float* gamma, const double* global_sums, double count,
                                 const double* local_sums, float* dgamma, float* dbeta, float* dw, float* dw_slabs,
                                 int N, int H, int W, int views, void* stream) {
    if (!x_nchw || !dz || !xo || !mean || !invstd || !global_sums || !dw || count <= 0 || views < 1 || N % views)
        return SM3_EINVAL;
    if (dw_slabs && (((uintptr_t)dw_slabs | (uintptr_t)dw) & 15)) return SM3_EALIGN;
    if (dtype != SM3_BF16 && dtype != SM3_F16 && dtype != SM3_F32) return SM3_EDTYPE;
    StemWgradParams p;
    if (int rc = stem_geometry(N, H, W, p.Ho, p.Wo, p.xblocks, p.tiles)) return rc;
    p.x = x_nchw; p.dz = (const char*)dz; p.xo = (const char*)xo;
    p.mean = mean; p.invstd = invstd; p.gamma = gamma; p.gsums = global_sums; p.lsums = local_sums;
    p.dgamma = dgamma; p.dbeta = dbeta; p.dw = dw; p.dw_slabs = dw_slabs; p.inv_count = 1.0 / count;
    p.N = N; p.H = H; p.W = W; p.n_per_view = N / views; p.views = views;
    if (dtype == SM3_F32) {
        const unsigned gridf = (unsigned)(p.tiles < 512 ? p.tiles : 512);
        hipLaunchKernelGGL(stem_wgrad_f32_kernel, dim3(gridf), dim3(256), 0, (hipStream_t)stream, p);
        SM3_CHECK_LAUNCH();
        return dw_slabs ? sm3_slab_reduce(dw_slabs, (int)gridf, 64 * 147, dw, 1, stream) : 0;
    }
    const unsigned grid = (unsigned)(p.tiles < SM3_STEM_WGRAD_SLABS ? p.tiles : SM3_STEM_WGRAD_SLABS);
    if (dtype == SM3_BF16)
        hipLaunchKernelGGL(stem_wgrad_kernel<bf16_t>, dim3(grid), dim3(256), 0, (hipStream_t)stream, p);
    else
        hipLaunchKernelGGL(stem_wgrad_kernel<f16_t>, dim3(grid), dim3(256), 0, (hipStream_t)stream, p);
    SM3_CHECK_LAUNCH();
    return dw_slabs ? sm3_slab_reduce(dw_slabs, (int)grid, 64 * 147, dw, 1, stream) : 0;
}

extern "C" int sm3_stem_image_cols(int W) { return W > 0 ? (W + 6 + 7) / 8 * 8 : SM3_EINVAL; }

extern "C" int sm3_stem_image_prep(int dtype, const float* x_view0, const float* x_view1, void* ximg, int n_per_view,
                                   int views, int H, int W, void* stream) {
    if (!x_view0 || !ximg || n_per_view <= 0 || H <= 0 || W <= 0 || views < 1 || views > 2 || (views == 2 && !x_view1))
        return SM3_EINVAL;
    if (dtype != SM3_BF16 && dtype != SM3_F16) return SM3_EDTYPE;
    if ((uintptr_t)ximg & 15) return SM3_EALIGN;
    const int Wp = sm3_stem_image_cols(W);
    const long chunks = (long)n_per_view * views * 3 * H * (Wp / 8);
    if (chunks * 16 >= 0xC0000000L) return SM3_EINVAL;
    const long blocks = (chunks + 255) / 256;
    if (dtype == SM3_BF16)
        hipLaunchKernelGGL(stem_image_prep_kernel<bf16_t>, dim3((unsigned)blocks), dim3(256), 0, (hipStream_t)stream, x_view0,
                           x_view1, (uint4*)ximg, n_per_view, H, W, Wp / 8, chunks);
    else
        hipLaunchKernelGGL(stem_image_prep_kernel<f16_t>, dim3((unsigned)blocks), dim3(256), 0, (hipStream_t)stream, x_view0,
                           x_view1, (uint4*)ximg, n_per_view, H, W, Wp / 8, chunks);
    SM3_CHECK_LAUNCH();
    return 0;
}

template <typename K>
static int stem16_allow_lds(K kern, int bytes) {
    static std::atomic<int> done[32];
    int dev = 0;
    if (hipGetDevice(&dev) != hipSuccess || dev < 0 || dev > 31) dev = 0;
    if (!done[dev].load(std::memory_order_acquire)) {
        hipError_t e = hipFuncSetAttribute(reinterpret_cast<const void*>(kern), hipFuncAttributeMaxDynamicSharedMemorySize, bytes);
        if (e != hipSuccess) return (int)e;
        done[dev].store(1, std::memory_order_release);
    }
    return 0;
}

extern "C" int sm3_stem_conv_fwd16(int dtype, const void* ximg, const void* w_stem, void* y, float* stat_partials, int N,
                                   int H, int W, void* stream) {
    if (!ximg || !w_stem || !y) return SM3_EINVAL;
    if (dtype != SM3_BF16 && dtype != SM3_F16) return SM3_EDTYPE;
    int Ho, Wo, xb;
    long tiles;
    if (int rc = stem_geometry(N, H, W, Ho, Wo, xb, tiles)) return rc;
    const int Wp = sm3_stem_image_cols(W);
    const long bytes = (long)N * 3 * H * Wp * 2;
    if (bytes >= 0xC0000000L) return SM3_EINVAL;
    if (tiles > 0x7fffffffL) return SM3_EINVAL;
    const TileDiv td{make_fastdiv((uint32_t)xb), make_fastdiv((uint32_t)Ho)};
    const unsigned grid = (unsigned)(tiles < 512 ? tiles : 512);
    if (dtype == SM3_BF16) {
        if (int rc = stem16_allow_lds(stem_fwd16_kernel<bf16_t>, FWD16_LDS)) return rc;
        hipLaunchKernelGGL(stem_fwd16_kernel<bf16_t>, dim3(grid), dim3(256), FWD16_LDS, (hipStream_t)stream, (const char*)ximg,
                           (uint32_t)bytes, (const uint4*)w_stem, (bf16_t*)y, stat_partials, H, Wp, Ho, Wo, td, (uint32_t)tiles);
    } else {
        if (int rc = stem16_allow_lds(stem_fwd16_kernel<f16_t>, FWD16_LDS)) return rc;
        hipLaunchKernelGGL(stem_fwd16_kernel<f16_t>, dim3(grid), dim3(256), FWD16_LDS, (hipStream_t)stream, (const char*)ximg,
                           (uint32_t)bytes, (const uint4*)w_stem, (f16_t*)y, stat_partials, H, Wp, Ho, Wo, td, (uint32_t)tiles);
    }
    SM3_CHECK_LAUNCH();
    return 0;
}

extern "C" int sm3_stem_wgrad_bn16(int dtype, const void* ximg, const void* dz, const void* xo, const float* mean,
                                   const float* invstd, const float* gamma, const double* global_sums, double count,
                                   const double* local_sums, float* dgamma, float* dbeta, float* dw, float* dw_slabs,
                                   int N, int H, int W, int views, void* stream) {
    if (!ximg || !dz || !xo || !mean || !invstd || !global_sums || !dw || count <= 0 || views < 1 || N % views)
        return SM3_EINVAL;
    if (dtype != SM3_BF16 && dtype != SM3_F16) return SM3_EDTYPE;
    if (dw_slabs && (((uintptr_t)dw_slabs | (uintptr_t)dw) & 15)) return SM3_EALIGN;
    StemWgrad16Params pp;
    StemWgradParams& p = pp.q;
    if (int rc = stem_geometry(N, H, W, p.Ho, p.Wo, p.xblocks, p.tiles)) return rc;
    pp.Wp = sm3_stem_image_cols(W);
    const long bytes = (long)N * 3 * H * pp.Wp * 2;
    if (bytes >= 0xC0000000L) return SM3_EINVAL;
    if (p.tiles > 0x7fffffffL) return SM3_EINVAL;
    pp.ximg = (const char*)ximg; pp.ximg_bytes = (uint32_t)bytes;
    pp.td = TileDiv{make_fastdiv((uint32_t)p.xblocks), make_fastdiv((uint32_t)p.Ho)};
    p.x = nullptr; p.dz = (const char*)dz; p.xo = (const char*)xo;
    p.mean = mean; p.invstd = invstd; p.gamma = gamma; p.gsums = global_sums; p.lsums = local_sums;
    p.dgamma = dgamma; p.dbeta = dbeta; p.dw = dw; p.dw_slabs = dw_slabs; p.inv_count = 1.0 / count;
    p.N = N; p.H = H; p.W = W; p.n_per_view = N / views; p.views = views;
    const unsigned grid = (unsigned)(p.tiles < SM3_STEM_WGRAD_SLABS ? p.tiles : SM3_STEM_WGRAD_SLABS);
    if (dtype == SM3_BF16)
        hipLaunchKernelGGL(stem_wgrad16_kernel<bf16_t>, dim3(grid), dim3(256), 0, (hipStream_t)stream, pp);
    else
        hipLaunchKernelGGL(stem_wgrad16_kernel<f16_t>, dim3(grid), dim3(256), 0, (hipStream_t)stream, pp);
    SM3_CHECK_LAUNCH();
    return dw_slabs ? sm3_slab_reduce(dw_slabs, (int)grid, 64 * 147, dw, 1, stream) : 0;
}

template <typename T>
static int stem_dgrad_launch(const StemDgradParams& p, hipStream_t stream) {
    static std::atomic<int> done[32];
    const int bytes = DgradCfg<T>::LDS;
    int dev = 0;
    if (hipGetDevice(&dev) != hipSuccess || dev < 0 || dev > 31) dev = 0;
    if (!done[dev].load(std::memory_order_acquire)) {
        hipError_t e = hipFuncSetAttribute(reinterpret_cast<const void*>(stem_dgrad_kernel<T>),
                                           hipFuncAttributeMaxDynamicSharedMemorySize, bytes);
        if (e != hipSuccess) return (int)e;
        done[dev].store(1, std::memory_order_release);
    }
    const long cap = sizeof(T) == 2 ? 512 : 256;
    const unsigned grid = (unsigned)(p.tiles < cap ? p.tiles : cap);
    hipLaunchKernelGGL(stem_dgrad_kernel<T>, dim3(grid), dim3(256), bytes, stream, p);
    SM3_CHECK_LAUNCH();
    return 0;
}

extern "C" int sm3_stem_dgrad_bn(int dtype, const void* dz, const void* xo, const float* mean, const float* invstd,
                                 const float* gamma, const double* global_sums, double count, const float* w_master,
                                 float* dx, int N, int H, int W, int views, void* stream) {
    if (!dz || !xo || !mean || !invstd || !global_sums || !w_master || !dx || !(count > 0) || views < 1 || N % views)
        return SM3_EINVAL;
    if (dtype != SM3_BF16 && dtype != SM3_F16 && dtype != SM3_F32) return SM3_EDTYPE;
    if ((((uintptr_t)dz) | ((uintptr_t)xo)) & 15) return SM3_EALIGN;
    StemDgradParams p;
    long tiles;
    if (int rc = stem_geometry(N, H, W, p.Ho, p.Wo, p.xblocks, tiles)) return rc;
    p.xblocks = (p.Wo + DG_J - 1) / DG_J;
    p.rchunks = (p.Ho + DG_RC - 1) / DG_RC;
    p.tiles = (long)N * p.rchunks * p.xblocks;
    p.dz = (const char*)dz; p.xo = (const char*)xo;
    p.mean = mean; p.invstd = invstd; p.gamma = gamma; p.gsums = global_sums; p.w = w_master; p.dx = dx;
    p.inv_count = 1.0 / count;
    p.H = H; p.W = W; p.n_per_view = N / views;
    if (dtype == SM3_BF16) return stem_dgrad_launch<bf16_t>(p, (hipStream_t)stream);
    if (dtype == SM3_F16) return stem_dgrad_launch<f16_t>(p, (hipStream_t)stream);
    return stem_dgrad_launch<float>(p, (hipStream_t)stream);
}
```

### skin-sm3_amd/sm3hip/_lib.py

```python
import ctypes as C
import os

_HERE = os.path.dirname(os.path.abspath(__file__))
LIB_PATH = os.environ.get("SM3_LIBRARY") or os.path.join(_HERE, "libsm3hip.so")

SM3_F32, SM3_BF16, SM3_F16 = 0, 1, 2
MAX_TAPS = 9


class ConvDesc(C.Structure):
    _fields_ = [
        ("dtype", C.c_int32),
        ("N", C.c_int32), ("Hi", C.c_int32), ("Wi", C.c_int32), ("Ci", C.c_int32),
        ("Ho", C.c_int32), ("Wo", C.c_int32), ("Co", C.c_int32),
        ("sy", C.c_int32), ("sx", C.c_int32),
        ("ntaps", C.c_int32),
        ("dy", C.c_int32 * MAX_TAPS), ("dx", C.c_int32 * MAX_TAPS), ("wtap", C.c_int32 * MAX_TAPS),
        ("w_row_stride", C.c_int32),
        ("Hout", C.c_int32), ("Wout", C.c_int32),
        ("osy", C.c_int32), ("osx", C.c_int32), ("ooy", C.c_int32), ("oox", C.c_int32),
    ]


class BnBwdFuse(C.Structure):
    _fields_ = [("relu_mask", C.c_void_p), ("x", C.c_void_p), ("mean", C.c_void_p), ("invstd", C.c_void_p),
                ("partials", C.c_void_p), ("partial_row_offset", C.c_int32), ("views", C.c_int32),
                ("partial_row_offset_view1", C.c_int32), ("addend_sp_h", C.c_int32), ("addend_sp_w", C.c_int32)]


class ConvSeg(C.Structure):
    _fields_ = [("x1", C.c_void_p), ("w1", C.c_void_p), ("Ci1", C.c_int32), ("w_view_stride", C.c_int64),
                ("w1_view_stride", C.c_int64), ("col_bias", C.c_void_p), ("views", C.c_int32)]


class BnApplySide(C.Structure):
    _fields_ = [("x", C.c_void_p), ("mean", C.c_void_p), ("invstd", C.c_void_p), ("gamma", C.c_void_p),
                ("global_sums", C.c_void_p), ("local_sums", C.c_void_p), ("dgamma", C.c_void_p), ("dbeta", C.c_void_p),
                ("dx", C.c_void_p)]


class WPrepItem(C.Structure):
    _fields_ = [("w", C.c_void_p), ("w_fwd", C.c_void_p), ("w_dgrad", C.c_void_p),
                ("Co", C.c_int32), ("taps", C.c_int32), ("Ci", C.c_int32), ("ld_fwd", C.c_int32)]


_P, _I, _L, _F, _D, _U = C.c_void_p, C.c_int, C.c_int64, C.c_float, C.c_double, C.c_uint32
_DESC = C.POINTER(ConvDesc)

SIGNATURES = {
    "sm3_abi_version": [],
    "sm3_conv_partial_rows": [_DESC],
    "sm3_conv_gather_gemm": [_DESC, _P, _P, _P, _P, _P, _P],
    "sm3_conv_dgrad_bnfuse": [_DESC, _P, _P, _P, _P, _P, _P],
    "sm3_conv_dgrad_seg_bnfuse": [_DESC, _P, _P, _P, _P, _P, _P, _P],
    "sm3_conv_gather_gemm_seg": [_DESC, _P, _P, _P, _P, _P, _P],
    "sm3_conv_seg_act": [_DESC, _P, _P, _P, _I, _P, _P, _P],
    "sm3_linbn_fold": [_P, _I, _I, _I, _P, _P],
    "sm3_p2p_mailbox_bytes": [],
    "sm3_p2p_max_elems": [],
    "sm3_p2p_max_world": [],
    "sm3_p2p_layout": [_I, _I, _I, _P, _P, _P, _P],
    "sm3_p2p_alloc": [_P, _P, _P],
    "sm3_p2p_open": [_P, _P],
    "sm3_p2p_close": [_P],
    "sm3_p2p_free": [_P],
    "sm3_p2p_allreduce_f64": [_P, _I, _P, _I, _I, C.c_uint64, _P, _D, _P],
    "sm3_linbn_scale_banks": [_I, _P, _I, _P, _P, _P, _P, _I, _P, _P, _P, _P, _I, _I, _P],
    "sm3_subsample_colsum_rows": [_L, _I, _I],
    "sm3_subsample_colsum": [_I, _P, _P, _P, _I, _I, _I, _I, _I, _I, _P],
    "sm3_conv_wgrad_cat": [_DESC, _P, _P, _P, _P, _I, _P, _I, _L, _L, _P],
    "sm3_bn_act_colsum_rows": [_L, _I, _I],
    "sm3_conv_wgrad_slabs": [_DESC, _P, _P, _P, _I, _I, _P, _P],
    "sm3_linbn_moments": [_P, _I, _L, _P, _P, _I, _P, _I, _I, _P],
    "sm3_bn_act_colsum": [_I, _P, _P, _P, _P, _I, _P, _P, _P, _L, _I, _I, _P],
    "sm3_conv_bn_act_fused": [_DESC, _P, _P, _P, _P, _P, _I, _P, _P, _I, _P],
    "sm3_linbn_fwd_stats": [_I, _P, _P, _P, _P, _P, _P, _I, _I, _I, _P],
    "sm3_linbn_stats": [_I, _P, _P, _P, _P, _P, _P, _I, _P, _P, _P, _D, _P, _I, _I, _I, _P],
    "sm3_linbn_coef": [_P, _D, _P, _P, _P, _P, _I, _I, _P],
    "sm3_linbn_banks": [_I, _P, _P, _P, _P, _P, _I, _I, _I, _P],
    "sm3_linbn_post": [_I, _P, _P, _P, _P, _P, _P, _P, _P, _P, _I, _I, _I, _P],
    "sm3_linbn_banks_post": [_I, _P, _P, _P, _P, _P, _P, _P, _P, _P, _P, _I, _I, _I, _P],
    "sm3_conv_bn_act_eval": [_DESC, _P, _P, _P, _P, _P, _I, _P, _P],
    "sm3_conv_bn_eval": [_DESC, _P, _P, _P, _P, _P, _P, _F, _P, _I, _P, _P],
    "sm3_conv_wgrad": [_DESC, _P, _P, _P, _P],
    "sm3_conv_wgrad_det": [_DESC, _P, _P, _P, _P, _I, _P],
    "sm3_slab_reduce": [_P, _I, _L, _P, _I, _P],
    "sm3_bn_stats_reduce": [_P, _I, _I, _P, _P, _I, _P],
    "sm3_bn_reduce_groups": [_I],
    "sm3_bn_finalize": [_P, _I, _I, _D, _I, _P, _P, _F, _F, _P, _P, _P, _P, _P, _P, _P, _P],
    "sm3_bn_eval_scale_shift": [_P, _P, _P, _P, _F, _I, _P, _P, _P],
    "sm3_bn_act": [_I, _P, _P, _P, _P, _I, _I, _P, _P, _L, _I, _I, _P],
    "sm3_bn_add_bn_act": [_I, _P, _P, _P, _P, _P, _P, _I, _P, _P, _L, _I, _I, _P],
    "sm3_bn_bwd_apply2": [_I, _P, _D, _P, _P, _L, _I, _I, _P],
    "sm3_bn_relu_maxpool_fwd": [_I, _P, _P, _P, _P, _P, _I, _I, _I, _I, _I, _P],
    "sm3_maxpool_bn_bwd_partial_rows": [_I, _I, _I, _I],
    "sm3_maxpool_bn_bwd": [_I, _P, _P, _P, _P, _P, _P, _P, _P, _P, _I, _I, _I, _I, _I, _P],
    "sm3_bn_bwd_partial_rows": [_L, _I],
    "sm3_bn_bwd_reduce": [_I, _P, _P, _P, _P, _P, _P, _P, _L, _I, _P, _I, _P],
    "sm3_bn_bwd_apply": [_I, _P, _P, _P, _P, _P, _P, _D, _P, _P, _P, _P, _L, _I, _I, _P],
    "sm3_stem_partial_rows": [_I, _I, _I],
    "sm3_stem_weight_prep": [_I, _P, _P, _P],
    "sm3_stem_weight_prep_if": [_I, _P, _P, _P, _P],
    "sm3_stem_conv_fwd": [_I, _P, _P, _P, _P, _I, _I, _I, _P],
    "sm3_stem_wgrad_bn": [_I, _P, _P, _P, _P, _P, _P, _P, _D, _P, _P, _P, _P, _P, _I, _I, _I, _I, _P],
    "sm3_stem_image_cols": [_I],
    "sm3_stem_image_prep": [_I, _P, _P, _P, _I, _I, _I, _I, _P],
    "sm3_stem_conv_fwd16": [_I, _P, _P, _P, _P, _I, _I, _I, _P],
    "sm3_stem_wgrad_bn16": [_I, _P, _P, _P, _P, _P, _P, _P, _D, _P, _P, _P, _P, _P, _I, _I, _I, _I, _P],
    "sm3_stem_dgrad_bn": [_I, _P, _P, _P, _P, _P, _P, _D, _P, _P, _I, _I, _I, _I, _P],
    "sm3_maxpool3x3s2_fwd": [_I, _P, _P, _P, _I, _I, _I, _I, _P],
    "sm3_maxpool3x3s2_bwd": [_I, _P, _P, _P, _I, _I, _I, _I, _P],
    "sm3_weight_prep_batch": [_I, _P, _I, _P],
    "sm3_weight_prep_batch_if": [_I, _P, _I, _P, _P],
    "sm3_weights_changed": [_P, _L, _P, _P, _P],
    "sm3_avgpool_fwd": [_I, _P, _P, _P, _I, _I, _I, _P],
    "sm3_avgpool_bwd": [_I, _P, _P, _I, _I, _I, _P],
    "sm3_weight_prep": [_I, _P, _I, _I, _I, _P, _I, _P, _P],
    "sm3_cast_from_f32": [_I, _P, _P, _L, _P],
    "sm3_cast_to_f32": [_I, _P, _P, _L, _P],
    "sm3_ntxent_logits": [_P, _I, _I, _F, _P, _P, _P, _P],
    "sm3_ntxent_logits_bwd": [_I, _P, _P, _P, _I, _I, _F, _P, _P],
    "sm3_ce_label0": [_P, _I, _I, _F, _P, _P, _P, _P],
    "sm3_ntxent_fused": [_I, _P, _I, _I, _F, _F, _P, _P, _P, _P],
    "sm3_normalize_rows": [_P, _I, _I, _P, _P, _P],
    "sm3_ntxent_rect": [_P, _I, _I, _I, _F, _F, _P, _P, _P, _P],
    "sm3_normalize_rows_bwd": [_I, _P, _P, _P, _P, _I, _I, _P, _P],
    "sm3_adamw": [_P, _P, _P, _P, _L, _F, _F, _F, _F, _F, _I, _F, _P, _P],
    "sm3_adamw_dynamic": [_P, _P, _P, _P, _L, _F, _F, _F, _F, _F, _F, _P, _P, _P, _P],
    "sm3_loss_scale_update": [_P, _P, _P, _P, _F, _F, _I, _P],
    "sm3_ntxent_fused_scaled": [_I, _P, _I, _I, _F, _F, _P, _P, _P, _P, _P],
    "sm3_ntxent_fused_batch": [_I, _I, _P, _I, _I, _F, _P, _P, _P, _P, _P, _P],
    "sm3_ema_update": [_P, _P, _L, _F, _P],
    "sm3_check_finite": [_P, _L, _P, _P],
    "sm3_aug_resized_crop": [_P, _I, _I, _I, _P, _P, _P, _I, _I, _P],
    "sm3_aug_resized_crop_ragged": [_P, _L, _P, _P, _P, _I, _P, _P, _P, _I, _P, _I, _I, _P],
    "sm3_aug_color_op": [_P, _I, _I, _I, _P, _P, _P, _P],
    "sm3_aug_finish": [_P, _I, _I, _I, _P, _P, _P, _P, _P, _P],
    "sm3_token_attention": [_I, _P, _P, _I, _I, _I, _I, _P],
    "sm3_add_layernorm": [_I, _P, _P, _P, _P, _F, _P, _L, _I, _P],
    "sm3_token_heads": [_I, _P, _P, _P, _P, _I, _P, _I, _I, _I, _I, _P],
    "sm3_mlc_attention_fwd": [_P, _P, _I, _I, _I, _I, _F, _U, _I, _P],
    "sm3_mlc_attention_bwd": [_P, _P, _P, _I, _I, _I, _I, _F, _U, _I, _P],
    "sm3_mlc_heads_fwd": [_P, _P, _P, _P, _I, _P, _I, _I, _I, _I, _I, _P],
    "sm3_mlc_add_ln_fwd": [_P, _P, _P, _P, _F, _F, _U, _P, _P, _L, _I, _P],
    "sm3_mlc_add_ln_bwd": [_P, _P, _P, _P, _P, _F, _U, _P, _P, _P, _P, _L, _I, _P],
    "sm3_mlc_bias_relu_drop_fwd": [_P, _P, _F, _U, _P, _P, _L, _I, _P],
    "sm3_mlc_relu_drop_bwd": [_P, _P, _F, _U, _P, _P, _L, _I, _P],
    "sm3_mlc_colsum": [_P, _P, _L, _I, _P],
    "sm3_mlc_ce": [_P, _P, _P, _I, _I, _I, _F, _P, _P, _P],
    "sm3_mlc_heads_bwd": [_P, _P, _P, _P, _I, _P, _P, _P, _I, _I, _I, _I, _I, _P],
    "sm3_mlc_kmeans_assign": [_P, _P, _P, _P, _P, _I, _I, _I, _P],
    "sm3_mlc_kmeans_update": [_P, _P, _P, _I, _I, _P],
    "sm3_mlc_colsum_det": [_P, _P, _P, _L, _I, _I, _P],
    "sm3_mlc_add_ln_bwd_det": [_P, _P, _P, _P, _P, _F, _U, _P, _P, _P, _P, _P, _L, _I, _P],
    "sm3_mlc_heads_bwd_det": [_P, _P, _P, _P, _I, _P, _P, _P, _P, _I, _I, _I, _I, _I, _P],
    "sm3_mlc_kmeans_assign_det": [_P, _P, _P, _P, _P, _P, _I, _I, _I, _P],
    "sm3_grouped_gemm": [_I, _P, _P, _P, _P, _I, _I, _I, _I, _P],
    "sm3_grouped_wgrad_det": [_I, _P, _P, _P, _P, _I, _I, _I, _I, _I, _P],
    "sm3_gconv_weight_prep": [_I, _P, _P, _P, _I, _I, _P, _P],
    "sm3_gconv_fwd": [_I, _P, _P, _P, _P, _I, _I, _I, _I, _I, _I, _P],
    "sm3_gconv_dgrad": [_I, _P, _P, _P, _I, _I, _I, _I, _I, _I, _P],
    "sm3_gconv_wgrad_slabs": [_I, _I, _I, _I, _I],
    "sm3_gconv_wgrad_det": [_I, _P, _P, _P, _P, _I, _I, _I, _I, _I, _I, _I, _P],
    "sm3_knn_vote": [_P, _L, _L, _L, _P, _I, _P, _I, _F, _P, _P, _P, _P],
    "sm3_cam_alpha": [_I, _P, _P, _I, _I, _I, _I, _P],
    "sm3_cam_maps": [_I, _P, _P, _P, _P, _I, _I, _I, _I, _I, _I, _I, _P],
    "sm3_attr_path": [_P, _P, _I, _P, _I, _L, _I, _I, _I, _P],
    "sm3_attr_noise": [_P, _P, _P, _I, _L, _I, _I, _I, C.c_uint64, _P],
    "sm3_attr_accumulate": [_P, _P, _I, _I, _L, _F, _I, _P],
    "sm3_attr_finish_blocks": [_I],
    "sm3_attr_finish": [_P, _P, _P, _I, _P, _P, _P, _P, _I, _I, _I, _I, _I, _P],
    "sm3_faith_rank_workspace": [_I, _I],
    "sm3_faith_rank": [_P, _P, _I, _I, _P, _L, _P],
    "sm3_faith_compose": [_P, _P, _I, _P, _L, _L, _P, _I, _I, _I, _I, _I, _I, _I, _P],
    "sm3_rise_table": [_P, _I, _I, _I, _I, _I, _I, _D, C.c_uint64, _P],
    "sm3_rise_compose": [_P, _P, _I, _P, _P, _I, _I, _I, _I, _I, _P],
    "sm3_rise_accumulate": [_P, _P, _P, _L, _L, _I, _I, _I, _I, _I, _I, _D, _P],
}

_lib = None


class SM3LibraryError(RuntimeError):
    pass


def load():
    global _lib
    if _lib is not None:
        return _lib
    if not os.path.exists(LIB_PATH):
        raise SM3LibraryError(
            f"{LIB_PATH} not found: build it with `make -C skin-sm3_amd/csrc` (or __graft_entry__.build()). "
            "The SM3 HIP path has no CPU fallback."
        )
    lib = C.CDLL(LIB_PATH)
    for name, argtypes in SIGNATURES.items():
        try:
            fn = getattr(lib, name)
        except AttributeError as e:
            raise SM3LibraryError(f"{LIB_PATH} does not export {name}") from e
        fn.argtypes = argtypes
        fn.restype = C.c_int
    _lib = lib
    return lib


def check(rc, what):
    if rc != 0:
        kind = {-1: "SM3_EINVAL", -2: "SM3_EALIGN", -3: "SM3_EDTYPE"}.get(rc, f"hipError {rc}")
        raise SM3LibraryError(f"{what} failed: {kind}")
```

### skin-sm3_amd/sm3hip/engine.py

```python
import os
from collections import OrderedDict
from contextlib import contextmanager

import torch

from . import ops
from ._lib import SM3_BF16, SM3_F16
from .plan import (TWO_PASS, BlockRec, EncoderCtx, ParamStore, ProjectorPlan, Rec, block_form, enc_mod_out_dim, enc_plan,
                   stage_of)
from .plan import EncoderPlan

BN_EPS = 1e-5
BN_MOMENTUM = 0.1


_LANE_POOL = {}


def lane_stream_pool(device, n):
    idx = device.index if device.index is not None else torch.cuda.current_device()
    pool = _LANE_POOL.setdefault(idx, [])
    if len(pool) >= n:
        return pool[:n]
    if os.environ.get("SM3_STREAM_CALIBRATE", "1") == "0" or not hasattr(torch.cuda, "_sleep"):
# ... 701 lines not shown
        for _ in range(5):
            h, w = (h - 1) // 2 + 1, (w - 1) // 2 + 1
            if (n_view * h * w) % 128:
                return False
        return True

    def encoder_forward(self, plan, x, train, feat_f32, feat_t, save=None, views=1, taps=None, keep=None):
        xs = list(x) if isinstance(x, (list, tuple)) else [x]
        if any(t.dtype != torch.float32 or t.dim() != 4 or t.shape[1] != 3 or t.shape != xs[0].shape for t in xs):
            raise ValueError("encoder input must be NCHW float32 with 3 channels")
        if len(xs) > 1 and not self.stem16:
            x = torch.cat(xs, 0)
        elif len(xs) == 1:
            x = xs[0]
        with self._views(views if train else 1):
            self._encoder_forward(plan, x, train, feat_f32, feat_t, save, taps, keep)

    stage_of = staticmethod(stage_of)

    def _encoder_forward(self, plan, x, train, feat_f32, feat_t, save, taps=None, keep_out=None):
        if self.stem16:
            xs = [t.contiguous() for t in (x if isinstance(x, (list, tuple)) else [x])]
            x = ops.stem_image_prep(self.dtype, xs)
            dev0 = xs[0].device
        else:
            x = x.contiguous()
            dev0 = x.device
        N, _, H, W = x.shape
        Ho, Wo = (H - 1) // 2 + 1, (W - 1) // 2 + 1
        saving = save is not None
        Hp, Wp = (Ho - 1) // 2 + 1, (Wo - 1) // 2 + 1
        p = torch.empty(N * Hp * Wp, 64, dtype=self.tdt, device=dev0)
        amax = torch.empty(N * Hp * Wp * 64, dtype=torch.uint8, device=dev0) if saving else None
        V = self._V
        sc = torch.empty(V * 64, dtype=torch.float32, device=dev0)
        sh = torch.empty(V * 64, dtype=torch.float32, device=dev0)
        xo, _, _, rs = self.conv_bn(plan.stem, plan.stem_bn, x, N, H, W, True, None, train, saving, apply=False,
                                    scale_shift=(sc, sh))
        if saving:
            rs.scale, rs.shift = sc, sh
        ops.bn_relu_maxpool_fwd(self.dtype, xo, sc, sh, p, N, Ho, Wo, 64, amax, views=V)
        del xo
        cur, h, w = p, Hp, Wp
        if taps is not None:
            taps["x"] = [p.clone()]
        block_recs = []
        kept = keep = None
        if keep_out is not None:
            keep = keep_out["stage"]
            if keep not in {stage_of(b) for b in plan.blocks}:
                raise ValueError(f"keep: no stage {keep!r} in this encoder")
        block_forward = self._basic_forward if plan.basic else self._bottleneck_forward
        for bi, blk in enumerate(plan.blocks):
            form = block_form(blk, bi, self, train, self.dtype, V, N, h, w) if saving else TWO_PASS
            cur, h, w, br = block_forward(blk, form, cur, N, h, w, train, saving)
            block_recs.append(br)
            if keep is not None and stage_of(blk) == keep:
                kept = (cur, h, w)
            if taps is not None:
                taps["x"].append(cur.clone())
        ops.avgpool_fwd(self.dtype, cur, feat_f32, feat_t, N, h * w, plan.out_dim)
        if keep_out is not None:
            keep_out["out"] = kept
        if saving:
            save.append(EncoderCtx(plan=plan, N=N, img_hw=(H, W), stem=rs, stem_hw=(Ho, Wo), argmax=amax,
                                   blocks=block_recs, last_hw=(h, w)))

    def _identity_branch(self, blk, cur, N, h, w, train, save):
        if "cd" not in blk:
            return cur, None, None, None
        if not (train or save):
            return self.conv_bn(blk["cd"], blk["bd"], cur, N, h, w, False, None, train)[0], None, None, None
        ra = (self._work("scale_d", 2 * 2048), self._work("shift_d", 2 * 2048))
        pend = [] if (train and self.stat_sync is not None) else None
        idn, _, _, rd = self.conv_bn(blk["cd"], blk["bd"], cur, N, h, w, False, None, train, save, apply=False,
                                     scale_shift=ra, pending=pend)
        return idn, ra, pend, rd

    def _basic_forward(self, blk, form, cur, N, h, w, train, save):
        y1, h1, w1, r1 = self.conv_bn(blk["c1"], blk["b1"], cur, N, h, w, True, None, train, save)
        idn, ra, pend, rd = self._identity_branch(blk, cur, N, h, w, train, save)
        y2, h2, w2, r2 = self.conv_bn(blk["c2"], blk["b2"], y1, N, h1, w1, True, idn, train, save, res_affine=ra,
                                      pending=pend)
        return y2, h2, w2, (BlockRec(form, r1, r2, rd=rd) if save else None)

    def _bottleneck_forward(self, blk, form, cur, N, h, w, train, save):
        V = self._V
        y1, h1, w1, r1 = self.conv_bn(blk["c1"], blk["b1"], cur, N, h, w, True, None, train, save)
        pp = blk["c3"].Ci
        cs = crow = None
        if form.lin:
            d2 = blk["c2"].fwd_desc(self.dtype, N, h1, w1)
            crow = ops.bn_act_colsum_rows(self.dtype, N * d2.Ho * d2.Wo // V, pp)
            cs = self._work("linbn_cs", V * crow * pp)
        y2, h2, w2, r2 = self.conv_bn(blk["c2"], blk["b2"], y1, N, h1, w1, True, None, train, save, colsum=cs)
        if form.lin:
            slabs, cap = self._slab_buf(pp * pp, V)
            ns = ops.conv_wgrad_slabs(self._lin_conv_desc(self.dtype, N, h2, w2, pp, pp), y2, y2, slabs, views=V, cap=cap)
            r2.gram = torch.empty(V * pp * pp, dtype=torch.float32, device=y2.device)
            r2.colsum = torch.empty(V * pp, dtype=torch.float64, device=y2.device)
            ops.linbn_moments(slabs, ns, pp * pp, r2.gram, views=V, colsum=cs, colsum_rows=crow, s_out=r2.colsum, p=pp)
        if form.join_fused:
            y3, h3, w3, rd, r3 = self.join_fused(blk, r2, y2, cur, N, h, w, h2, w2)
        else:
            idn, ra, pend, rd = self._identity_branch(blk, cur, N, h, w, train, save)
            if form.conv3_fused:
                y3, h3, w3, r3 = self.conv3_bn3_fused(blk["c3"], blk["b3"], r2, y2, idn, N, h2, w2)
            else:
                y3, h3, w3, r3 = self.conv_bn(blk["c3"], blk["b3"], y2, N, h2, w2, True, idn, train, save, res_affine=ra,
                                              pending=pend)
                if form.lin:
                    r3.linbn = True
        return y3, h3, w3, (BlockRec(form, r1, r2, r3, rd) if save else None)

    def encoder_backward(self, ctx, dfeat, last_view=True, taps=None, dx_out=None, params=True, stop_at=None):
        with self._params_backward(params):
            return self._encoder_backward(ctx, dfeat, last_view, taps, dx_out, stop_at)

    def _stop_block(self, ctx, stop_at):
        names = [stage_of(b) for b in ctx.plan.blocks]
        if stop_at not in names or names[-1] == stop_at:
            raise ValueError(f"stop_at: {stop_at!r} is not a stage below the last one of this encoder")
        if not ctx.stem.frozen_stats:
            raise NotImplementedError("stop_at: eval-mode (frozen-statistics) contexts only")
        return max(i for i, n in enumerate(names) if n == stop_at) + 1

    def _encoder_backward(self, ctx, dfeat, last_view, taps, dx_out, stop_at=None):
        plan, N = ctx.plan, ctx.N
        stop_bi = self._stop_block(ctx, stop_at) if stop_at is not None else -1
        h, w = ctx.last_hw
        dcur = torch.empty(N * h * w, plan.out_dim, dtype=self.tdt, device=dfeat.device)
        ops.avgpool_bwd(self.dtype, dfeat, dcur, N, h * w, plan.out_dim)
        fr = None
        if taps is not None:
            taps["g"] = [None] * (len(plan.blocks) + 1)
            taps["g_pre_relu"] = [False] * (len(plan.blocks) + 1)
        block_backward = self._basic_backward if plan.basic else self._bottleneck_backward
        for bi in range(len(plan.blocks) - 1, -1, -1):
            blk = plan.blocks[bi]
            unfused_in = bi == stop_bi
            if taps is not None:
                taps["g"][bi + 1], taps["g_pre_relu"][bi + 1] = dcur.clone(), fr is not None
            prev = ctx.blocks[bi - 1].join if bi > 0 and not unfused_in else None
            dcur, fr = block_backward(ctx.blocks[bi], dcur, fr, prev)
            if unfused_in:
                return dcur
            if last_view and "cd" in blk and bi > 0:
                stage = blk["c1"].name.rsplit(".", 2)[0]
                self._notify(stage + ".", stage + ".")
        if taps is not None:
            taps["g"][0] = dcur.clone()
        Ho, Wo = ctx.stem_hw
        rs = ctx.stem
        dz = torch.empty(N * Ho * Wo, 64, dtype=self.tdt, device=dfeat.device)
        prow = ops.maxpool_bn_bwd_partial_rows(N, Ho, Wo, rs.V)
        part = self._work("fz_partials", rs.V * prow * 2 * 64)
        ops.maxpool_bn_bwd(self.dtype, ctx.argmax, dcur, rs.xo, rs.scale, rs.shift, rs.mean, rs.invstd, dz, part,
                           N, Ho, Wo, 64, views=rs.V)
        lsums, gsums, count = self._bn_backward_sums(rs, part, prow)
        gamma = self._bn_affine(rs.bu)[0]
        if not self._data_only:
            dgamma, dbeta = self._bn_affine(rs.bu, grad=True)
            wg = ops.stem_wgrad_bn16 if isinstance(rs.x_in, ops.StemImage) else ops.stem_wgrad_bn
            wg(self.dtype, rs.x_in, dz, rs.xo, rs.mean, rs.invstd, gamma, gsums, count, lsums, dgamma, dbeta,
               self._g(rs.cu.name + ".weight"), views=rs.V,
               slabs=self._work("stem_slabs", ops.STEM_WGRAD_SLABS * 64 * 147) if self.det_wgrad else None)
        if dx_out is not None:
            ops.stem_dgrad_bn(self.dtype, dz, rs.xo, rs.mean, rs.invstd, gamma, gsums, count,
                              self._p(rs.cu.name + ".weight"), dx_out, views=rs.V)
        if last_view:
            self._notify(plan.prefix + "conv1", plan.prefix + "layer1.")

    def _basic_backward(self, br, dcur, fr, prev):
        dxd = dz = None
        if br.rd is not None:
            dx2, dxd = self.bn_backward_join(br.r2, br.rd, dcur, fused_rows=fr)
        else:
            dx2, dz = self.bn_backward(br.r2, dcur, keep_dz=True, fused_rows=fr)
        dy1, fr1 = self.conv_backward(br.r2, dx2, fuse=br.r1)
        del dx2
        return self._block_input_backward(br, dy1, fr1, dcur, dz, dxd, prev)

    def _bottleneck_backward(self, br, dcur, fr, prev):
        r1, r2, r3, rd = br.r1, br.r2, br.r3, br.rd
        dxd = dz = None
        if br.form.lin:
            prow, bpart = self._phase1(r3, dcur, fr)
            dy2, fr2, dxd = self.conv3_backward_linbn(br, dcur, bpart, prow)
            if rd is None:
                dz = dcur
        else:
            if rd is not None:
                dx3, dxd = self.bn_backward_join(r3, rd, dcur, fused_rows=fr)
            else:
                dx3, dz = self.bn_backward(r3, dcur, keep_dz=True, fused_rows=fr)
            dy2, fr2 = self.conv_backward(r3, dx3, fuse=r2)
            del dx3
        dx2, _ = self.bn_backward(r2, dy2, keep_dz=False, fused_rows=fr2)
        dy1, fr1 = self.conv_backward(r2, dx2, fuse=r1)
        del dx2, dy2
        return self._block_input_backward(br, dy1, fr1, dcur, dz, dxd, prev)

    def _block_input_backward(self, br, dy1, fr1, dcur, dz, dxd, prev):
        r1, rd = br.r1, br.rd
        dx1, _ = self.bn_backward(r1, dy1, keep_dz=False, fused_rows=fr1)
        if rd is None:
            return self.conv_backward(r1, dx1, addend=dz, fuse=prev)
        cd = rd.cu
        if br.form.lin_d:
            Cd, Cin = cd.Co, cd.Ci
            dd = cd.compact_dgrad_desc(self.dtype, rd.N, rd.Ho, rd.Wo)
            if cd.stride == 2:
                dsp = torch.empty(rd.N * rd.Ho * rd.Wo, Cin, dtype=self.tdt, device=dcur.device)
                ops.conv_gemm_seg(dd, dcur, dxd["wa"], dxd["x1"], dxd["hn"], dxd["const"], dsp, None, views=rd.V,
                                  w_view_stride=Cin * Cd, w1_view_stride=Cin * Cin)
                return self.conv_backward(r1, dx1, addend=dsp, fuse=prev, addend_sparse=(rd.Ho, rd.Wo))
            din, _ = self.conv_backward(r1, dx1)
            ops.conv_gemm_seg(dd, dcur, dxd["wa"], dxd["x1"], dxd["hn"], dxd["const"], din, din, views=rd.V,
                              w_view_stride=Cin * Cd, w1_view_stride=Cin * Cin)
            return din, None
        if br.form.sparse_join and prev is not None:
            self._wgrad(cd, rd, dxd)
            hs, ws = rd.Ho, rd.Wo
            dd = cd.compact_dgrad_desc(self.dtype, rd.N, hs, ws)
            dsp = torch.empty(rd.N * hs * ws, cd.Ci, dtype=self.tdt, device=dxd.device)
            ops.conv_gemm(dd, dxd, cd.w_dgrad, dsp, None, None)
            return self.conv_backward(r1, dx1, addend=dsp, fuse=prev, addend_sparse=(hs, ws))
        din, _ = self.conv_backward(r1, dx1)
        self.conv_backward(rd, dxd, into=din)
        return din, None

    def projector_forward(self, plan, x_t, M, train, z_out, save=None):
        saving = save is not None
        h, _, _, r0 = self.conv_bn(plan.l0, plan.b1, x_t, M, 1, 1, True, None, train, saving)
        h, _, _, r3 = self.conv_bn(plan.l3, plan.b4, h, M, 1, 1, True, None, train, saving)
        r6 = self.conv_bn(plan.l6, plan.b7, h, M, 1, 1, False, None, train, saving, out_f32=True, y_out=z_out)[3]
        if saving:
            save.append((r0, r3, r6))

    def projector_backward(self, recs, dz, addend=None, into=None):
        r0, r3, r6 = recs
        dx, _ = self.bn_backward(r6, dz, keep_dz=False)
        d, fr = self.conv_backward(r6, dx, fuse=r3)
        dx, _ = self.bn_backward(r3, d, keep_dz=False, fused_rows=fr)
        d, fr = self.conv_backward(r3, dx, fuse=r0)
        dx, _ = self.bn_backward(r0, d, keep_dz=False, fused_rows=fr)
        if into is not None:
            return self.conv_backward(r0, dx, into=into)[0]
        return self.conv_backward(r0, dx, addend=addend)[0]

    @staticmethod
    def cross_pairs(style):
        return {0: [(0, 0), (1, 1)], 1: [(0, 1), (1, 0)], 2: [(0, 0), (0, 1), (1, 0), (1, 1)]}[style]

    def forward(self, views, style=0, train=True, want_grad=True, metadata=None):
        first = next(iter(views.values()))[0]
        dev = first.device
        self.prepare(dev)
        self.refresh_weights(defer_lanes=self._lane_streams(dev) is not None and self.lane_cross)
        B = first.shape[0]
        saved = {"B": B, "style": style} if want_grad else None
        sv = (lambda: []) if want_grad else (lambda: None)
        zs, feats = OrderedDict(), {}
        streams = self._lane_streams(dev)
        lane_cross = self._cross_in_lanes(streams)
        pairs = self.cross_pairs(style) if self.cross is not None else []
        zc = [self._share(torch.empty(2 * B, self.module.proj_dim, dtype=torch.float32, device=dev), streams) for _ in pairs] \
            if lane_cross else []
        cross_recs = {}
        for key, (plan, proj) in self.branches.items():
            imgs = views[key]
            with self.lane(key, streams):
                self.prep_lane(key)
            for im in imgs:
                self._share(im, streams)
            f32 = self._share(torch.empty(2 * B, plan.out_dim, dtype=torch.float32, device=dev), streams)
            ft = self._share(torch.empty(2 * B, plan.out_dim, dtype=self.tdt, device=dev), streams)
            ctxs = [None, None] if want_grad else None
            pair = (self.pair_views and train and len(imgs) == 2 and imgs[0].shape == imgs[1].shape
                    and self.pair_ok(B, imgs[0].shape[2], imgs[0].shape[3])
                    and 2 * B * ((imgs[0].shape[2] - 1) // 2 + 1) * ((imgs[0].shape[3] - 1) // 2 + 1)
                    * 64 * ops._sz(self.dtype) < 0xC0000000)
            if pair:
                with self.lane(key, streams):
                    tmp = [] if want_grad else None
                    self.encoder_forward(plan, [imgs[0], imgs[1]], train, f32, ft, tmp, views=2)
                    if want_grad:
                        ctxs = [tmp[0]]
            for v in (() if pair else (0, 1)):
                with self.lane(key, streams):
                    tmp = [] if want_grad else None
                    self.encoder_forward(plan, imgs[v], train, f32[v * B:(v + 1) * B], ft[v * B:(v + 1) * B], tmp)
                    if want_grad:
                        ctxs[v] = tmp[0]
            feats[key] = (f32, ft)
            precs = sv()
            with self.lane(key, streams):
                if proj is not None:
                    z = torch.empty(2 * B, self.module.proj_dim, dtype=torch.float32, device=dev)
                    self.projector_forward(proj, ft, 2 * B, train, z, precs)
                    zs[key] = self._share(z, streams)
                if lane_cross:
                    side = 0 if key == "derm" else 1
                    for ci, ab in enumerate(pairs):
                        rec = sv()
                        self.projector_forward(self.cross[side], ft[ab[side] * B:(ab[side] + 1) * B], B, train,
                                               zc[ci][side * B:(side + 1) * B], rec)
                        cross_recs[(ci, side)] = rec
            if want_grad:
                saved[key] = {"enc": ctxs, "proj": precs[0] if proj is not None else None}
        self._join(streams)
        for k in list(self._lane_prep):
            self.prep_lane(k)
        cross_saved = []
        if lane_cross:
            for ci, (a, b) in enumerate(pairs):
                zs[f"cross{ci}"] = zc[ci]
                if want_grad:
                    cross_saved.append((a, b, cross_recs[(ci, 0)][0], cross_recs[(ci, 1)][0]))
# ... 128 lines not shown
```

### skin-sm3_amd/sm3hip/ops.py

```python
import ctypes as C

import torch

from . import _lib
from ._lib import ConvDesc, SM3_BF16, SM3_F16, SM3_F32, check

TORCH_DTYPE = {SM3_F32: torch.float32, SM3_BF16: torch.bfloat16, SM3_F16: torch.float16}
K_CHUNK = {SM3_F32: 32, SM3_BF16: 64, SM3_F16: 64}


_PROFILER = None


def set_profiler(p):
    global _PROFILER
    _PROFILER = p


class _prof:
    __slots__ = ("tag", "flops", "nbytes", "start")

    def __init__(self, tag, flops=0.0, nbytes=0.0):
        self.tag, self.flops, self.nbytes, self.start = tag, flops, nbytes, None

# ... 788 lines not shown
    for t, n in ((scale, "scale"), (shift, "shift"), (save_mean, "save_mean"), (save_invstd, "save_invstd")):
        _chk(t, torch.float32, n)
        if t is not None and t.numel() < views * Cn:
            raise ValueError(f"{n} too small")
    _chk(sums, torch.float64, "sums"); _chk(nbt, torch.int64, "num_batches_tracked")
    if sums.numel() < views * groups * 2 * Cn:
        raise ValueError("bn_finalize: sums too small for groups")
    with _prof("bn_finalize", 0.0, 40.0 * Cn):
        check(_lib.load().sm3_bn_finalize(_ptr(sums), groups, views, float(count), Cn, _ptr(gamma), _ptr(beta), eps,
                                          momentum, _ptr(running_mean), _ptr(running_var), _ptr(nbt), _ptr(scale),
                                          _ptr(shift), _ptr(save_mean), _ptr(save_invstd), _stream()), "sm3_bn_finalize")


def bn_eval_scale_shift(gamma, beta, running_mean, running_var, eps, Cn, scale, shift):
    for t in (gamma, beta, running_mean, running_var, scale, shift):
        _chk(t, torch.float32)
    check(_lib.load().sm3_bn_eval_scale_shift(_ptr(gamma), _ptr(beta), _ptr(running_mean), _ptr(running_var), eps,
                                              Cn, _ptr(scale), _ptr(shift), _stream()), "sm3_bn_eval_scale_shift")


def subsample_colsum_rows(dtype, rows, Cn):
    return _lib.load().sm3_subsample_colsum_rows(rows, Cn, dtype)


def subsample_colsum(dtype, x, y, colsum, N, H, W, Cn, stride, views=1):
    tdt = TORCH_DTYPE[dtype]
    _chk(x, tdt, "x"); _chk(y, tdt, "y"); _chk(colsum, torch.float32, "colsum")
    Hs, Ws = (H - 1) // stride + 1, (W - 1) // stride + 1
    if x.numel() != N * H * W * Cn or (y is not None and y.numel() != N * Hs * Ws * Cn) or N % views:
        raise ValueError("subsample_colsum: size mismatch")
    if colsum.numel() < views * subsample_colsum_rows(dtype, N // views * Hs * Ws, Cn) * Cn:
        raise ValueError("subsample_colsum: colsum too small")
    with _prof("subsample", 0.0, _sz(dtype) * N * Hs * Ws * Cn * (2 if y is not None else 1)):
        check(_lib.load().sm3_subsample_colsum(dtype, _ptr(x), _ptr(y), _ptr(colsum), N, H, W, Cn, stride, views, _stream()),
              "sm3_subsample_colsum")


def bn_act_colsum_rows(dtype, rows, Cn):
    return _lib.load().sm3_bn_act_colsum_rows(rows, Cn, dtype)


def bn_act(dtype, x, scale, shift, residual, relu, y, rows, Cn, out_f32=False, mask=None, views=1, colsum=None):
    tdt = TORCH_DTYPE[dtype]
    _chk(x, tdt, "x"); _chk(residual, tdt, "residual"); _chk(scale, torch.float32); _chk(shift, torch.float32)
    _chk(y, torch.float32 if out_f32 else tdt, "y")
    n = views * rows * Cn
    if x.numel() != n or y.numel() != n or (residual is not None and residual.numel() != n):
        raise ValueError("bn_act: size mismatch")
    if scale.numel() < views * Cn or shift.numel() < views * Cn:
        raise ValueError("bn_act: scale/shift too small")
    _chk(mask, torch.uint8, "mask")
    if mask is not None and mask.numel() != n // (16 // _sz(dtype)):
        raise ValueError("bn_act: mask size mismatch")
    tag = "bn_act"
    if _PROFILER is not None and getattr(_PROFILER, "detail", False):
        tag += f"|rows{views * rows}_C{Cn}_res{int(residual is not None)}"
    _chk(colsum, torch.float32, "colsum")
    if colsum is not None and (out_f32 or colsum.numel() < views * bn_act_colsum_rows(dtype, rows, Cn) * Cn):
        raise ValueError("bn_act: colsum needs the storage dtype and [views][colsum_rows][C] floats")
    with _prof(tag, 0.0, _sz(dtype) * n * (2 if residual is None else 3)):
        if colsum is not None:
            check(_lib.load().sm3_bn_act_colsum(dtype, _ptr(x), _ptr(scale), _ptr(shift), _ptr(residual), int(relu),
                                                _ptr(y), _ptr(mask), _ptr(colsum), rows, Cn, views, _stream()),
                  "sm3_bn_act_colsum")
        else:
            check(_lib.load().sm3_bn_act(dtype, _ptr(x), _ptr(scale), _ptr(shift), _ptr(residual), int(relu),
                                         int(out_f32), _ptr(y), _ptr(mask), rows, Cn, views, _stream()), "sm3_bn_act")


def bn_add_bn_act(dtype, x, scale, shift, x2, scale2, shift2, relu, y, rows, Cn, mask=None, views=1):
    tdt = TORCH_DTYPE[dtype]
    for t in (x, x2, y):
        _chk(t, tdt)
    for t in (scale, shift, scale2, shift2):
        _chk(t, torch.float32)
        if t.numel() < views * Cn:
            raise ValueError("bn_add_bn_act: scale/shift too small")
    n = views * rows * Cn
    if x.numel() != n or x2.numel() != n or y.numel() != n:
        raise ValueError("bn_add_bn_act: size mismatch")
    _chk(mask, torch.uint8, "mask")
    if mask is not None and mask.numel() != n // (16 // _sz(dtype)):
        raise ValueError("bn_add_bn_act: mask size mismatch")
    tag = "bn_act"
    if _PROFILER is not None and getattr(_PROFILER, "detail", False):
        tag += f"|rows{views * rows}_C{Cn}_res2"
    with _prof(tag, 0.0, _sz(dtype) * n * 3):
        check(_lib.load().sm3_bn_add_bn_act(dtype, _ptr(x), _ptr(scale), _ptr(shift), _ptr(x2), _ptr(scale2),
                                            _ptr(shift2), int(relu), _ptr(y), _ptr(mask), rows, Cn, views, _stream()),
              "sm3_bn_add_bn_act")


def bn_bwd_apply2(dtype, dz, count, side_a, side_b, rows, Cn, views=1):
    tdt = TORCH_DTYPE[dtype]
    _chk(dz, tdt, "dz")
    n = views * rows * Cn
    if dz.numel() != n:
        raise ValueError("bn_bwd_apply2: dz size mismatch")
    sides = []
    for sd in (side_a, side_b):
        for k in ("x", "dx"):
            _chk(sd[k], tdt, k)
            if sd[k].numel() != n:
                raise ValueError(f"bn_bwd_apply2: {k} size mismatch")
        for k in ("mean", "invstd", "gamma", "dgamma", "dbeta"):
            _chk(sd.get(k), torch.float32, k)
        for k in ("gsums", "lsums"):
            _chk(sd.get(k), torch.float64, k)
            if sd.get(k) is not None and sd[k].numel() < views * 2 * Cn:
                raise ValueError("bn_bwd_apply2: sums too small")
        if sd["mean"].numel() < views * Cn or sd["invstd"].numel() < views * Cn:
            raise ValueError("bn_bwd_apply2: mean/invstd too small")
        a = _lib.BnApplySide()
        a.x, a.mean, a.invstd, a.dx = sd["x"].data_ptr(), sd["mean"].data_ptr(), sd["invstd"].data_ptr(), sd["dx"].data_ptr()
        a.global_sums = sd["gsums"].data_ptr()
        for k, f in (("gamma", "gamma"), ("lsums", "local_sums"), ("dgamma", "dgamma"), ("dbeta", "dbeta")):
            setattr(a, f, sd[k].data_ptr() if sd.get(k) is not None else None)
        sides.append(a)
    tag = "bn_bwd_apply"
    if _PROFILER is not None and getattr(_PROFILER, "detail", False):
        tag += f"|rows{views * rows}_C{Cn}_dual"
    with _prof(tag, 0.0, _sz(dtype) * n * 5):
        check(_lib.load().sm3_bn_bwd_apply2(dtype, _ptr(dz), float(count), C.byref(sides[0]), C.byref(sides[1]), rows, Cn,
                                            views, _stream()), "sm3_bn_bwd_apply2")


def bn_relu_maxpool_fwd(dtype, x, scale, shift, y, N, H, W, Cn, argmax=None, views=1):
    tdt = TORCH_DTYPE[dtype]
    _chk(x, tdt, "x"); _chk(y, tdt, "y"); _chk(scale, torch.float32); _chk(shift, torch.float32); _chk(argmax, torch.uint8)
    Ho, Wo = (H - 1) // 2 + 1, (W - 1) // 2 + 1
    if x.numel() != N * H * W * Cn or y.numel() != N * Ho * Wo * Cn or N % views:
        raise ValueError("bn_relu_maxpool_fwd: size mismatch")
    if scale.numel() < views * Cn or shift.numel() < views * Cn:
        raise ValueError("bn_relu_maxpool_fwd: scale/shift too small")
    if argmax is not None and argmax.numel() != y.numel():
        raise ValueError("bn_relu_maxpool_fwd: argmax size mismatch")
    with _prof("bn_relu_maxpool", 0.0, _sz(dtype) * (x.numel() + y.numel()) + (y.numel() if argmax is not None else 0)):
        check(_lib.load().sm3_bn_relu_maxpool_fwd(dtype, _ptr(x), _ptr(scale), _ptr(shift), _ptr(y), _ptr(argmax), N, H, W,
                                                  Cn, views, _stream()), "sm3_bn_relu_maxpool_fwd")


def maxpool_bn_bwd_partial_rows(N, H, W, views=1):
    return _lib.load().sm3_maxpool_bn_bwd_partial_rows(N, H, W, views)


def maxpool_bn_bwd(dtype, argmax, dy, x, scale, shift, mean, invstd, dz, partials, N, H, W, Cn, views=1):
    tdt = TORCH_DTYPE[dtype]
    _chk(argmax, torch.uint8); _chk(dy, tdt, "dy"); _chk(x, tdt, "x"); _chk(dz, tdt, "dz"); _chk(partials, torch.float32)
    for t in (scale, shift, mean, invstd):
        _chk(t, torch.float32)
        if t.numel() < views * Cn:
            raise ValueError("maxpool_bn_bwd: per-channel vector too small")
    Ho, Wo = (H - 1) // 2 + 1, (W - 1) // 2 + 1
    if x.numel() != N * H * W * Cn or dz.numel() != x.numel() or dy.numel() != N * Ho * Wo * Cn or \
            argmax.numel() != dy.numel() or N % views:
        raise ValueError("maxpool_bn_bwd: size mismatch")
    if partials.numel() < views * maxpool_bn_bwd_partial_rows(N, H, W, views) * 2 * Cn:
        raise ValueError("maxpool_bn_bwd: partials too small")
    with _prof("maxpool_bn_bwd", 0.0, _sz(dtype) * (2 * x.numel() + dy.numel()) + argmax.numel()):
        check(_lib.load().sm3_maxpool_bn_bwd(dtype, _ptr(argmax), _ptr(dy), _ptr(x), _ptr(scale), _ptr(shift), _ptr(mean),
                                             _ptr(invstd), _ptr(dz), _ptr(partials), N, H, W, Cn, views, _stream()),
              "sm3_maxpool_bn_bwd")


def bn_bwd_partial_rows(rows, Cn):
    return _lib.load().sm3_bn_bwd_partial_rows(rows, Cn)


def bn_bwd_reduce(dtype, dy, y, x, mean, invstd, dz, rows, Cn, partials, mask=None, views=1):
    tdt = TORCH_DTYPE[dtype]
    n = views * rows * Cn
    for t, nm in ((dy, "dy"), (y, "y"), (x, "x"), (dz, "dz")):
        _chk(t, tdt, nm)
        if t is not None and t.numel() != n:
            raise ValueError(f"bn_bwd_reduce: {nm} size mismatch")
    _chk(partials, torch.float32)
    if partials.numel() < views * bn_bwd_partial_rows(rows, Cn) * 2 * Cn:
        raise ValueError("bn_bwd_reduce: partials too small")
    _chk(mask, torch.uint8, "mask")
    if mask is not None and mask.numel() != n // (16 // _sz(dtype)):
        raise ValueError("bn_bwd_reduce: mask size mismatch")
    if x is not None and (mean.numel() < views * Cn or invstd.numel() < views * Cn):
        raise ValueError("bn_bwd_reduce: mean/invstd too small")
    reads = 1 + (x is not None) + (1 if (y is not None and mask is None) else 0) + (1 if dz is not None else 0)
    with _prof("bn_bwd_reduce", 0.0, _sz(dtype) * n * reads + (n // 8 if mask is not None else 0)):
        check(_lib.load().sm3_bn_bwd_reduce(dtype, _ptr(dy), _ptr(y), _ptr(mask), _ptr(x), _ptr(mean), _ptr(invstd),
                                            _ptr(dz), rows, Cn, _ptr(partials), views, _stream()), "sm3_bn_bwd_reduce")


def bn_bwd_apply(dtype, dz, x, mean, invstd, gamma, gsums, count, lsums, dgamma, dbeta, dx, rows, Cn, views=1):
    tdt = TORCH_DTYPE[dtype]
    for t, n in ((dz, "dz"), (x, "x"), (dx, "dx")):
        _chk(t, tdt, n)
        if t.numel() != views * rows * Cn:
            raise ValueError(f"bn_bwd_apply: {n} size mismatch")
    _chk(gsums, torch.float64); _chk(lsums, torch.float64)
    _chk(dgamma, torch.float32); _chk(dbeta, torch.float32); _chk(gamma, torch.float32)
    if gsums.numel() < views * 2 * Cn or (lsums is not None and lsums.numel() < views * 2 * Cn):
        raise ValueError("bn_bwd_apply: sums too small")
    tag = "bn_bwd_apply"
    if _PROFILER is not None and getattr(_PROFILER, "detail", False):
        tag += f"|rows{views * rows}_C{Cn}"
    with _prof(tag, 0.0, _sz(dtype) * views * rows * Cn * 3):
        check(_lib.load().sm3_bn_bwd_apply(dtype, _ptr(dz), _ptr(x), _ptr(mean), _ptr(invstd), _ptr(gamma),
                                           _ptr(gsums), float(count), _ptr(lsums), _ptr(dgamma), _ptr(dbeta), _ptr(dx),
                                           rows, Cn, views, _stream()), "sm3_bn_bwd_apply")


STEM_KDIRECT = 176


def stem_partial_rows(N, H, W):
    return _lib.load().sm3_stem_partial_rows(N, H, W)


def stem_weight_prep(dtype, w_master, w_stem, only_if=None):
    _chk(w_master, torch.float32, "w_master"); _chk(w_stem, TORCH_DTYPE[dtype], "w_stem"); _chk(only_if, torch.int32, "only_if")
    if w_master.numel() != 64 * 147 or w_stem.numel() != 64 * STEM_KDIRECT:
        raise ValueError("stem_weight_prep: size mismatch")
    check(_lib.load().sm3_stem_weight_prep_if(dtype, _ptr(w_master), _ptr(w_stem), _ptr(only_if), _stream()),
          "sm3_stem_weight_prep_if")


def stem_conv_fwd(dtype, x_nchw, w_stem, y, partials=None):
    _chk(x_nchw, torch.float32, "x"); _chk(w_stem, TORCH_DTYPE[dtype], "w_stem"); _chk(y, TORCH_DTYPE[dtype], "y")
    _chk(partials, torch.float32, "partials")
    N, Cc, H, W = x_nchw.shape
    Ho, Wo = (H - 1) // 2 + 1, (W - 1) // 2 + 1
    if Cc != 3 or w_stem.numel() != 64 * STEM_KDIRECT or y.numel() != N * Ho * Wo * 64:
        raise ValueError("stem_conv_fwd: size mismatch")
    if partials is not None and partials.numel() < stem_partial_rows(N, H, W) * 2 * 64:
        raise ValueError("stem_conv_fwd: partials too small")
    M = N * Ho * Wo
    with _prof("stem_conv_fwd", 2.0 * M * 64 * 147, 4.0 * x_nchw.numel() + _sz(dtype) * y.numel()):
        check(_lib.load().sm3_stem_conv_fwd(dtype, _ptr(x_nchw), _ptr(w_stem), _ptr(y), _ptr(partials), N, H, W, _stream()),
              "sm3_stem_conv_fwd")


STEM_WGRAD_SLABS = 768


class StemImage:
    __slots__ = ("t", "shape")

    def __init__(self, t, shape):
        self.t, self.shape = t, tuple(shape)

    def record_stream(self, st):
        self.t.record_stream(st)


def stem_image_cols(W):
    return (W + 6 + 7) // 8 * 8


def stem_image_prep(dtype, views):
    x0 = views[0]
    x1 = views[1] if len(views) > 1 else None
    _chk(x0, torch.float32, "x0"); _chk(x1, torch.float32, "x1")
    if x0.dim() != 4 or x0.shape[1] != 3 or (x1 is not None and x1.shape != x0.shape) or len(views) > 2:
        raise ValueError("stem_image_prep: NCHW fp32 views of equal shape")
    B, _, H, W = x0.shape
    V = len(views)
    out = torch.empty(V * B, 3, H, stem_image_cols(W), dtype=TORCH_DTYPE[dtype], device=x0.device)
    with _prof("stem_image_prep", 0.0, 4.0 * V * x0.numel() + _sz(dtype) * out.numel()):
        check(_lib.load().sm3_stem_image_prep(dtype, _ptr(x0), _ptr(x1), _ptr(out), B, V, H, W, _stream()),
              "sm3_stem_image_prep")
    return StemImage(out, (V * B, 3, H, W))


def stem_conv_fwd16(dtype, img, w_stem, y, partials=None):
    tdt = TORCH_DTYPE[dtype]
    _chk(img.t, tdt, "ximg"); _chk(w_stem, tdt, "w_stem"); _chk(y, tdt, "y"); _chk(partials, torch.float32, "partials")
    N, Cc, H, W = img.shape
    Ho, Wo = (H - 1) // 2 + 1, (W - 1) // 2 + 1
    if Cc != 3 or w_stem.numel() != 64 * STEM_KDIRECT or y.numel() != N * Ho * Wo * 64 or \
            img.t.numel() != N * 3 * H * stem_image_cols(W):
        raise ValueError("stem_conv_fwd16: size mismatch")
    if partials is not None and partials.numel() < stem_partial_rows(N, H, W) * 2 * 64:
        raise ValueError("stem_conv_fwd16: partials too small")
    M = N * Ho * Wo
    with _prof("stem_conv_fwd", 2.0 * M * 64 * 147, _sz(dtype) * (img.t.numel() + y.numel())):
        check(_lib.load().sm3_stem_conv_fwd16(dtype, _ptr(img.t), _ptr(w_stem), _ptr(y), _ptr(partials), N, H, W, _stream()),
              "sm3_stem_conv_fwd16")


def stem_wgrad_bn16(dtype, img, dz, xo, mean, invstd, gamma, gsums, count, lsums, dgamma, dbeta, dw, views=1, slabs=None):
    tdt = TORCH_DTYPE[dtype]
    _chk(img.t, tdt, "ximg"); _chk(dz, tdt, "dz"); _chk(xo, tdt, "xo"); _chk(dw, torch.float32, "dw")
    for t in (mean, invstd, gamma, dgamma, dbeta):
        _chk(t, torch.float32)
    _chk(gsums, torch.float64); _chk(lsums, torch.float64); _chk(slabs, torch.float32, "slabs")
    N, Cc, H, W = img.shape
    Ho, Wo = (H - 1) // 2 + 1, (W - 1) // 2 + 1
    if Cc != 3 or dz.numel() != N * Ho * Wo * 64 or xo.numel() != dz.numel() or dw.numel() < 64 * 147 or N % views or \
            img.t.numel() != N * 3 * H * stem_image_cols(W):
        raise ValueError("stem_wgrad_bn16: size mismatch")
    if mean.numel() < views * 64 or invstd.numel() < views * 64 or gsums.numel() < views * 128 or \
            (lsums is not None and lsums.numel() < views * 128):
        raise ValueError("stem_wgrad_bn16: per-channel vector too small")
    if slabs is not None and slabs.numel() < STEM_WGRAD_SLABS * 64 * 147:
        raise ValueError("stem_wgrad_bn16: slab workspace too small")
    M = N * Ho * Wo
    with _prof("stem_wgrad_bn", 2.0 * M * 64 * 147, _sz(dtype) * (img.t.numel() + 2 * dz.numel())):
        check(_lib.load().sm3_stem_wgrad_bn16(dtype, _ptr(img.t), _ptr(dz), _ptr(xo), _ptr(mean), _ptr(invstd), _ptr(gamma),
                                              _ptr(gsums), float(count), _ptr(lsums), _ptr(dgamma), _ptr(dbeta), _ptr(dw),
                                              _ptr(slabs), N, H, W, views, _stream()), "sm3_stem_wgrad_bn16")


def stem_dgrad_bn(dtype, dz, xo, mean, invstd, gamma, gsums, count, w_master, dx, views=1):
    tdt = TORCH_DTYPE[dtype]
    _chk(dz, tdt, "dz"); _chk(xo, tdt, "xo"); _chk(dx, torch.float32, "dx"); _chk(w_master, torch.float32, "w")
    for t in (mean, invstd, gamma):
        _chk(t, torch.float32)
    _chk(gsums, torch.float64)
    if dx.dim() != 4 or dx.shape[1] != 3:
        raise ValueError("stem_dgrad_bn: dx must be [N, 3, H, W]")
    N, _, H, W = dx.shape
    Ho, Wo = (H - 1) // 2 + 1, (W - 1) // 2 + 1
    if dz.numel() != N * Ho * Wo * 64 or xo.numel() != dz.numel() or w_master.numel() != 64 * 147 or views < 1 or N % views:
        raise ValueError("stem_dgrad_bn: size mismatch")
    if mean.numel() < views * 64 or invstd.numel() < views * 64 or gsums.numel() < views * 128 or \
            (gamma is not None and gamma.numel() < 64):
        raise ValueError("stem_dgrad_bn: per-channel vector too small")
    M = N * Ho * Wo
    with _prof("stem_dgrad_bn", 2.0 * M * 64 * 147, 2.0 * _sz(dtype) * dz.numel() + 4.0 * dx.numel()):
        check(_lib.load().sm3_stem_dgrad_bn(dtype, _ptr(dz), _ptr(xo), _ptr(mean), _ptr(invstd), _ptr(gamma), _ptr(gsums),
                                            float(count), _ptr(w_master), _ptr(dx), N, H, W, views, _stream()),
              "sm3_stem_dgrad_bn")


def cam_alpha(dtype, g, alpha, N, HW, C):
    _chk(g, TORCH_DTYPE[dtype], "g"); _chk(alpha, torch.float32, "alpha")
    T = alpha.numel() // (N * C) if N * C > 0 else 0
    if T < 1 or alpha.numel() != T * N * C or g.numel() != T * N * HW * C:
        raise ValueError("cam_alpha: g [T, N, HW, C] and alpha [T, N, C] do not match")
    with _prof("cam_alpha", float(g.numel()), _sz(dtype) * g.numel() + 4.0 * alpha.numel()):
        check(_lib.load().sm3_cam_alpha(dtype, _ptr(g), _ptr(alpha), T, N, HW, C, _stream()), "sm3_cam_alpha")


def cam_maps(dtype, a, alpha, low, maps, N, h, w, C):
    _chk(a, TORCH_DTYPE[dtype], "a")
    for t, n in ((alpha, "alpha"), (low, "low"), (maps, "maps")):
        _chk(t, torch.float32, n)
    T = alpha.numel() // (N * C) if N * C > 0 else 0
    if maps.dim() != 4 or tuple(maps.shape[:2]) != (N, T) or tuple(low.shape) != (N, T, h, w):
        raise ValueError("cam_maps: low must be [N, T, h, w] and maps [N, T, H, W]")
    if T < 1 or alpha.numel() != T * N * C or a.numel() != N * h * w * C:
        raise ValueError("cam_maps: a [N, h*w, C] and alpha [T, N, C] do not match")
    H, W = maps.shape[2], maps.shape[3]
    with _prof("cam_maps", 2.0 * N * h * w * C * T, _sz(dtype) * a.numel() + 4.0 * (low.numel() + maps.numel())):
        check(_lib.load().sm3_cam_maps(dtype, _ptr(a), _ptr(alpha), _ptr(low), _ptr(maps), N, T, h, w, C, H, W, _stream()),
              "sm3_cam_maps")


def _attr_rows(x, name):
    _chk(x, torch.float32, name)
    if x.dim() < 2 or x.shape[0] < 1:
        raise ValueError(f"{name} must be [N, ...]")
    return x.shape[0], x.numel() // x.shape[0]


def attr_path(x, base, out, k0, steps):
    N, E = _attr_rows(x, "x")
    _chk(base, torch.float32, "base"); _chk(out, torch.float32, "out")
    c = out.shape[0] if out.dim() > 1 else 0
    if c < 1 or out.numel() != c * N * E or base.numel() not in (E, N * E):
        raise ValueError("attr_path: x [N, E], base [1 | N, E] and out [c, N, E] do not match")
    with _prof("attr_path", 3.0 * out.numel(), 4.0 * (x.numel() + base.numel() + out.numel())):
        check(_lib.load().sm3_attr_path(_ptr(x), _ptr(base), base.numel() // E, _ptr(out), N, E, k0, c, steps, _stream()),
              "sm3_attr_path")


def attr_noise(x, sigma, out, k0, seed, stride=1):
    N, E = _attr_rows(x, "x")
    _chk(sigma, torch.float32, "sigma"); _chk(out, torch.float32, "out")
    c = out.shape[0] if out.dim() > 1 else 0
    if c < 1 or out.numel() != c * N * E or sigma.numel() != N:
        raise ValueError("attr_noise: x [N, E], sigma [N] and out [c, N, E] do not match")
    if not 0 <= seed < 2 ** 64:
        raise ValueError("attr_noise: seed must fit 64 bits")
    with _prof("attr_noise", 2.0 * out.numel(), 4.0 * (x.numel() + out.numel())):
        check(_lib.load().sm3_attr_noise(_ptr(x), _ptr(sigma), _ptr(out), N, E, k0, c, stride, seed, _stream()),
              "sm3_attr_noise")


def attr_accumulate(g, acc, weight, squared=False):
    N, E = _attr_rows(acc, "acc")
    _chk(g, torch.float32, "g")
    c = g.numel() // (N * E)
    if c < 1 or g.numel() != c * N * E:
        raise ValueError("attr_accumulate: g [c, N, E] and acc [N, E] do not match")
    with _prof("attr_accumulate", 2.0 * g.numel(), 4.0 * (g.numel() + 2 * acc.numel())):
        check(_lib.load().sm3_attr_accumulate(_ptr(g), _ptr(acc), c, N, E, float(weight), int(bool(squared)), _stream()),
              "sm3_attr_accumulate")


def attr_finish(acc, x, base, attr, maps, sums, mode):
    if acc.dim() != 5 or attr.shape != acc.shape:
        raise ValueError("attr_finish: acc and attr must be [T, N, C, H, W]")
    T, N, Cc, H, W = acc.shape
    for t, n in ((acc, "acc"), (attr, "attr"), (maps, "maps")):
        _chk(t, torch.float32, n)
    _chk(sums, torch.float64, "sums")
    if tuple(maps.shape) != (T, N, H, W) or tuple(sums.shape) != (T, N) or mode not in (0, 1):
        raise ValueError("attr_finish: maps must be [T, N, H, W], sums [T, N], mode 0 or 1")
    base_n = 1
    if mode == 0:
        _chk(x, torch.float32, "x"); _chk(base, torch.float32, "base")
        E = Cc * H * W
        if x.numel() != N * E or base.numel() not in (E, N * E):
            raise ValueError("attr_finish: x [N, C, H, W] and base [1 | N, C, H, W] do not match acc")
        base_n = base.numel() // E
    else:
        x = base = None
    lib = _lib.load()
    blocks = lib.sm3_attr_finish_blocks(H * W)
    if blocks < 1:
        raise ValueError("attr_finish: empty images")
    partials = torch.empty(T * N * blocks, dtype=torch.float64, device=acc.device)
    with _prof("attr_finish", 4.0 * acc.numel(), 4.0 * (2 * acc.numel() + maps.numel())):
        check(lib.sm3_attr_finish(_ptr(acc), _ptr(x), _ptr(base), base_n, _ptr(attr), _ptr(maps), _ptr(sums), _ptr(partials),
                                  T, N, Cc, H * W, mode, _stream()), "sm3_attr_finish")


FAITH_RANK_WORKSPACE = 256 << 20


def faith_rank(maps, ranks):
    _chk(maps, torch.float32, "maps"); _chk(ranks, torch.int32, "ranks")
    if maps.dim() < 1 or maps.shape != ranks.shape or maps.numel() < 1:
        raise ValueError("faith_rank: maps [..., HW] fp32 and ranks [..., HW] int32 must have the same, non-empty shape")
    HW = maps.shape[-1]
    rows = maps.numel() // HW
    lib = _lib.load()
    one = lib.sm3_faith_rank_workspace(1, HW)
    if one < 1:
        raise ValueError(f"faith_rank: HW = {HW} is out of range")
    group = max(1, min(rows, FAITH_RANK_WORKSPACE // one))
    ws = torch.empty(group * one, dtype=torch.uint8, device=maps.device)
    m2, r2 = maps.view(rows, HW), ranks.view(rows, HW)
    with _prof("faith_rank", 0.0, 4.0 * 2 * maps.numel() + 8.0 * 8 * maps.numel()):
        for r0 in range(0, rows, group):
            g = min(group, rows - r0)
            check(lib.sm3_faith_rank(_ptr(m2[r0:]), _ptr(r2[r0:]), g, HW, _ptr(ws), ws.numel(), _stream()), "sm3_faith_rank")


def faith_compose(x, base, ranks, out, k0, steps, invert):
    N, E = _attr_rows(x, "x")
    _chk(base, torch.float32, "base"); _chk(out, torch.float32, "out")
    if x.dim() != 4 or x.shape[1] != 3 or out.dim() != 6 or ranks.dim() != 4:
        raise ValueError("faith_compose: x [N, 3, H, W], ranks [N, T, H, W], out [c, T, N, 3, H, W]")
    H, W = x.shape[2:]
    c, T = out.shape[:2]
    if not ranks.is_cuda or ranks.dtype != torch.int32 or tuple(ranks.shape) != (N, T, H, W) or ranks.stride(3) != 1 or \
            ranks.stride(2) != W:
        raise ValueError("faith_compose: ranks must be int32 [N, T, H, W] on the GPU with contiguous pixels")
    if c < 1 or tuple(out.shape) != (c, T, N, 3, H, W) or base.numel() not in (E, N * E):
        raise ValueError("faith_compose: x [N, 3, H, W], base [1 | N, 3, H, W] and out [c, T, N, 3, H, W] do not match")
    with _prof("faith_compose", 0.0, 4.0 * (T * x.numel() + T * base.numel() + ranks.numel() + out.numel())):
# ... 393 lines not shown
```

Before: 4611.

## Route maxpool backward into stem wgrad to skip materializing dz

When the stem weight gradient runs with the 16-bit image path and no input gradient is needed, the maxpool/BN backward kernel now only computes the BN statistics partials and skips writing the dz tensor. The stem wgrad kernel recomputes the routed maxpool gradient and ReLU mask on the fly from argmax, dy, and the BN scale/shift. This removes one full write and one read of the stem-resolution activation gradient. The cost is redundant argmax/dy gathers inside the wgrad kernel, more registers and shared memory there. The maxpool backward kernel also gains 32-bit offset math for small sizes and a transposed shared-memory reduction layout.

```diff
diff --git a/include/sm3_hip.h b/include/sm3_hip.h
--- a/include/sm3_hip.h
+++ b/include/sm3_hip.h
@@ -168,7 +168,7 @@
 int sm3_stem_wgrad_bn16(int dtype, const void* ximg, const void* dz, const void* xo, const float* mean, const float* invstd,
                         const float* gamma, const double* global_sums, double count, const double* local_sums,
                         float* dgamma, float* dbeta, float* dw, float* dw_slabs, int N, int H, int W, int views,
-                        void* stream);
+                        void* stream, const uint8_t* argmax, const void* dy, const float* scale, const float* shift);
 int sm3_stem_dgrad_bn(int dtype, const void* dz, const void* xo, const float* mean, const float* invstd, const float* gamma,
                       const double* global_sums, double count, const float* w_master, float* dx, int N, int H, int W,
                       int views, void* stream);
diff --git a/skin-sm3_amd/csrc/pool.hip b/skin-sm3_amd/csrc/pool.hip
--- a/skin-sm3_amd/csrc/pool.hip
+++ b/skin-sm3_amd/csrc/pool.hip
@@ -1,3 +1,5 @@
+#include <type_traits>
+
 #include "common.h"
 
 namespace {
@@ -175,7 +177,7 @@
     }
 }
 
-template <typename T>
+template <typename T, bool SMALL>
 __global__ __launch_bounds__(256) void maxpool_bn_bwd_kernel(const uint8_t* __restrict__ argmax, const T* __restrict__ dy,
                                                              const T* __restrict__ x, const float* __restrict__ scale,
                                                              const float* __restrict__ shift,
@@ -185,9 +187,14 @@
                                                              int Wo, int n_per_view, int64_t rows, int tbx, int tby,
                                                              const FastDiv div_hw, const FastDiv div_w) {
     constexpr int E = ElemTraits<T>::kPer16B;
-    __shared__ float sred[256 * 2 * 8];
+    using Off = std::conditional_t<SMALL, uint32_t, int64_t>;
+    constexpr Off kT = (Off)sizeof(T);
+    __shared__ float sred[2 * 8 * 256];
     const int tx = threadIdx.x % tbx, ty = threadIdx.x / tbx;
     const int cv = blockIdx.x * tbx + tx;
+    const char* __restrict__ xb = reinterpret_cast<const char*>(x);
+    const char* __restrict__ dyb = reinterpret_cast<const char*>(dy);
+    char* __restrict__ dzb = reinterpret_cast<char*>(dz);
     const bool active = (cv * E < C) && (ty < tby);
     const int view = blockIdx.z;
     float s1[E], s2[E];
@@ -208,11 +215,14 @@
             uint4 xu[U], du[U][4];
             unsigned au[U][4][2];
             int selfs[U][4];
-            int64_t pixs[U];
+            Off xoff[U];
+            bool live[U];
+            const Off cvo = (Off)cv * E;
 #pragma unroll
             for (int u = 0; u < U; ++u) {
                 const int64_t r = r0 + u * rstep;
-                pixs[u] = -1;
+                live[u] = false;
+                xoff[u] = 0;
                 xu[u] = make_uint4(0, 0, 0, 0);
 #pragma unroll
                 for (int w = 0; w < 4; ++w) selfs[u][w] = -1;
@@ -220,9 +230,10 @@
                 const uint32_t nl = fdiv((uint32_t)r, div_hw);
                 const uint32_t rem = (uint32_t)r - nl * div_hw.d;
                 const int iy = (int)fdiv(rem, div_w), ix = (int)(rem - (uint32_t)iy * div_w.d);
-                const int64_t n = (int64_t)view * n_per_view + nl;
-                pixs[u] = (int64_t)view * rows + r;
-                xu[u] = ldg16<true>(x + pixs[u] * C + (int64_t)cv * E);
+                const Off n = (Off)view * (Off)n_per_view + (Off)nl;
+                live[u] = true;
+                xoff[u] = (((Off)view * (Off)rows + (Off)r) * (Off)C + cvo) * kT;
+                xu[u] = ldg16<true>(xb + xoff[u]);
                 const int oy_lo = iy / 2, oy_hi = min(Ho - 1, (iy + 1) / 2);
                 const int ox_lo = ix / 2, ox_hi = min(Wo - 1, (ix + 1) / 2);
 #pragma unroll
@@ -230,7 +241,7 @@
                     const int oy = oy_lo + (w >> 1), ox = ox_lo + (w & 1);
                     if (oy > oy_hi || ox > ox_hi) continue;
                     selfs[u][w] = (iy - (oy * 2 - 1)) * 3 + (ix - (ox * 2 - 1));
-                    const int64_t o = ((n * Ho + oy) * Wo + ox) * C + (int64_t)cv * E;
+                    const Off o = ((n * (Off)Ho + (Off)oy) * (Off)Wo + (Off)ox) * (Off)C + cvo;
                     if constexpr (E == 8) {
                         const uint2 q = *reinterpret_cast<const uint2*>(argmax + o);
                         au[u][w][0] = q.x;
@@ -239,12 +250,12 @@
                         au[u][w][0] = *reinterpret_cast<const unsigned*>(argmax + o);
                         au[u][w][1] = 0;
                     }
-                    du[u][w] = *reinterpret_cast<const uint4*>(dy + o);
+                    du[u][w] = *reinterpret_cast<const uint4*>(dyb + o * kT);
                 }
             }
 #pragma unroll
             for (int u = 0; u < U; ++u) {
-                if (pixs[u] < 0) continue;
+                if (!live[u]) continue;
                 float g[E];
 #pragma unroll
                 for (int e = 0; e < E; ++e) g[e] = 0.f;
@@ -262,7 +273,7 @@
 #pragma unroll
                 for (int e = 0; e < E; ++e) g[e] = (xv[e] * sc[e] + sh[e] > ElemTraits<T>::kReluBit) ? g[e] : 0.f;
                 const uint4 packed = pack16<T>(g);
-                stg16<true>(dz + pixs[u] * C + (int64_t)cv * E, packed);
+                if (dz) stg16<true>(dzb + xoff[u], packed);
                 float gr[E];
                 unpack16<T>(packed, gr);
 #pragma unroll
@@ -273,20 +284,19 @@
             }
         }
     }
-    float* mine = sred + threadIdx.x * 2 * E;
 #pragma unroll
     for (int e = 0; e < E; ++e) {
-        mine[e] = s1[e];
-        mine[E + e] = s2[e];
+        sred[e * 256 + threadIdx.x] = s1[e];
+        sred[(E + e) * 256 + threadIdx.x] = s2[e];
     }
     __syncthreads();
     if (ty == 0 && cv * E < C) {
         for (int j = 1; j < tby; ++j) {
-            const float* o = sred + (j * tbx + tx) * 2 * E;
+            const float* o = sred + j * tbx + tx;
 #pragma unroll
             for (int e = 0; e < E; ++e) {
-                s1[e] += o[e];
-                s2[e] += o[E + e];
+                s1[e] += o[e * 256];
+                s2[e] += o[(E + e) * 256];
             }
         }
         float* pv = partials + (int64_t)view * gridDim.y * 2 * C;
@@ -523,8 +533,8 @@
     const int Ho = (H + 2 - 3) / 2 + 1, Wo = (W + 2 - 3) / 2 + 1;
     const int64_t total = (int64_t)N * Ho * Wo * (C / E);
     if (total >= 0x7fffffffLL) return SM3_EINVAL;
+    hipStream_t st = (hipStream_t)stream;
     const unsigned g = grid_for(total, 256, 1 << 20);
-    hipStream_t st = (hipStream_t)stream;
     const PixDiv dv = make_pixdiv(C / E, Wo, Ho);
     DISPATCH_T(dtype,
                hipLaunchKernelGGL(bn_relu_maxpool_fwd_kernel<float>, dim3(g), dim3(256), 0, st, (const float*)x, scale, shift, (float*)y, argmax, N, H, W, C, Ho, Wo, N / views, (uint32_t)total, dv),
@@ -532,6 +542,21 @@
                hipLaunchKernelGGL(bn_relu_maxpool_fwd_kernel<f16_t>, dim3(g), dim3(256), 0, st, (const f16_t*)x, scale, shift, (f16_t*)y, argmax, N, H, W, C, Ho, Wo, N / views, (uint32_t)total, dv));
     SM3_CHECK_LAUNCH();
     return 0;
+}
+
+namespace {
+template <typename T>
+void launch_maxpool_bn_bwd(bool small, dim3 grid, hipStream_t st, const uint8_t* argmax, const void* dy, const void* x,
+                           const float* scale, const float* shift, const float* mean, const float* invstd, void* dz,
+                           float* partials, int H, int W, int C, int Ho, int Wo, int n_per_view, int64_t rows, int tbx, int tby,
+                           FastDiv dhw, FastDiv dw) {
+    if (small)
+        hipLaunchKernelGGL((maxpool_bn_bwd_kernel<T, true>), grid, dim3(256), 0, st, argmax, (const T*)dy, (const T*)x, scale, shift,
+                           mean, invstd, (T*)dz, partials, H, W, C, Ho, Wo, n_per_view, rows, tbx, tby, dhw, dw);
+    else
+        hipLaunchKernelGGL((maxpool_bn_bwd_kernel<T, false>), grid, dim3(256), 0, st, argmax, (const T*)dy, (const T*)x, scale, shift,
+                           mean, invstd, (T*)dz, partials, H, W, C, Ho, Wo, n_per_view, rows, tbx, tby, dhw, dw);
+}
 }
 
 extern "C" int sm3_maxpool_bn_bwd_partial_rows(int N, int H, int W, int views) {
@@ -543,7 +568,7 @@
 extern "C" int sm3_maxpool_bn_bwd(int dtype, const uint8_t* argmax, const void* dy, const void* x, const float* scale,
                                   const float* shift, const float* mean, const float* invstd, void* dz,
                                   float* partials, int N, int H, int W, int C, int views, void* stream) {
-    if (!argmax || !dy || !x || !scale || !shift || !mean || !invstd || !dz || !partials) return SM3_EINVAL;
+    if (!argmax || !dy || !x || !scale || !shift || !mean || !invstd || !partials) return SM3_EINVAL;
     if (N <= 0 || H <= 0 || W <= 0 || C <= 0 || views < 1 || N % views) return SM3_EINVAL;
     if (!SM3_DTYPE_OK(dtype)) return SM3_EDTYPE;
     const int E = dtype == SM3_F32 ? 4 : 8;
@@ -560,10 +585,11 @@
     hipStream_t st = (hipStream_t)stream;
     const FastDiv dhw = make_fastdiv((uint32_t)(H * W)), dw = make_fastdiv((uint32_t)W);
     dim3 grid(gx, gy, views);
-    DISPATCH_T(dtype,
-               hipLaunchKernelGGL(maxpool_bn_bwd_kernel<float>, grid, dim3(256), 0, st, argmax, (const float*)dy, (const float*)x, scale, shift, mean, invstd, (float*)dz, partials, H, W, C, Ho, Wo, N / views, rows, tbx, tby, dhw, dw),
-               hipLaunchKernelGGL(maxpool_bn_bwd_kernel<bf16_t>, grid, dim3(256), 0, st, argmax, (const bf16_t*)dy, (const bf16_t*)x, scale, shift, mean, invstd, (bf16_t*)dz, partials, H, W, C, Ho, Wo, N / views, rows, tbx, tby, dhw, dw),
-               hipLaunchKernelGGL(maxpool_bn_bwd_kernel<f16_t>, grid, dim3(256), 0, st, argmax, (const f16_t*)dy, (const f16_t*)x, scale, shift, mean, invstd, (f16_t*)dz, partials, H, W, C, Ho, Wo, N / views, rows, tbx, tby, dhw, dw));
+    const bool small = (rows * views + 1) * (int64_t)(gx * tbx * E) * (dtype == SM3_F32 ? 4 : 2) < 0xffffffffLL;
+    DISPATCH_T(dtype,
+               launch_maxpool_bn_bwd<float>(small, grid, st, argmax, dy, x, scale, shift, mean, invstd, dz, partials, H, W, C, Ho, Wo, N / views, rows, tbx, tby, dhw, dw),
+               launch_maxpool_bn_bwd<bf16_t>(small, grid, st, argmax, dy, x, scale, shift, mean, invstd, dz, partials, H, W, C, Ho, Wo, N / views, rows, tbx, tby, dhw, dw),
+               launch_maxpool_bn_bwd<f16_t>(small, grid, st, argmax, dy, x, scale, shift, mean, invstd, dz, partials, H, W, C, Ho, Wo, N / views, rows, tbx, tby, dhw, dw));
     SM3_CHECK_LAUNCH();
     return 0;
 }
diff --git a/skin-sm3_amd/csrc/stem.hip b/skin-sm3_amd/csrc/stem.hip
--- a/skin-sm3_amd/csrc/stem.hip
+++ b/skin-sm3_amd/csrc/stem.hip
@@ -453,14 +453,18 @@
     uint32_t ximg_bytes;
     int Wp;
     TileDiv td;
+    const uint8_t* argmax;
+    const char* dyp;
+    const float *scale, *shift;
+    int Hq, Wq;
 };
 
-template <typename T>
+template <typename T, bool ROUTED>
 __global__ __launch_bounds__(256, 3) void stem_wgrad16_kernel(const StemWgrad16Params pp) {
     const StemWgradParams& p = pp.q;
     __shared__ __attribute__((aligned(16))) char sPatch[2 * PATCH16];
     __shared__ __attribute__((aligned(16))) char sD[128 * 128];
-    __shared__ __attribute__((aligned(16))) float sCoef[3][64];
+    __shared__ __attribute__((aligned(16))) float sCoef[ROUTED ? 5 : 3][64];
     const int tid = threadIdx.x, lane = tid & 63, wave = __builtin_amdgcn_readfirstlane(tid >> 6);
     const int cb = wave & 1, kb0 = 3 * (wave >> 1);
 
@@ -509,6 +513,10 @@
                 sCoef[0][c] = k0c;
                 sCoef[1][c] = qc;
                 sCoef[2][c] = qc * p.mean[view * 64 + c] - k0c * k1c;
+                if constexpr (ROUTED) {
+                    sCoef[3][c] = pp.scale[view * 64 + c];
+                    sCoef[4][c] = pp.shift[view * 64 + c];
+                }
             }
             __syncthreads();
         }
@@ -520,29 +528,94 @@
             *reinterpret_cast<float4*>(cC + e) = *reinterpret_cast<const float4*>(&sCoef[2][ch * 8 + e]);
         }
         const long pix0 = ((long)tl.n * p.Ho + tl.oy) * p.Wo + tl.x0;
-#pragma unroll
-        for (int kb = 0; kb < 4; kb += 2) {
-            uint4 gu[2], xu[2];
-#pragma unroll
-            for (int k = 0; k < 2; ++k) {
-                const int row = r0 + 32 * (kb + k);
-                const bool ok = tl.x0 + row < p.Wo;
-                gu[k] = ok ? ldg16<true>(p.dz + ((pix0 + row) * 64 + ch * 8) * 2) : make_uint4(0, 0, 0, 0);
-                xu[k] = ok ? ldg16<true>(p.xo + ((pix0 + row) * 64 + ch * 8) * 2) : make_uint4(0, 0, 0, 0);
-            }
-#pragma unroll
-            for (int k = 0; k < 2; ++k) {
-                const int row = r0 + 32 * (kb + k);
-                uint4 out = make_uint4(0, 0, 0, 0);
-                if (tl.x0 + row < p.Wo) {
-                    float g[8], xv[8];
-                    unpack16<T>(gu[k], g);
-                    unpack16<T>(xu[k], xv);
-#pragma unroll
-                    for (int e = 0; e < 8; ++e) g[e] = cA[e] * g[e] - cB[e] * xv[e] + cC[e];
-                    out = pack16<T>(g);
+        if constexpr (!ROUTED) {
+#pragma unroll
+            for (int kb = 0; kb < 4; kb += 2) {
+                uint4 gu[2], xu[2];
+#pragma unroll
+                for (int k = 0; k < 2; ++k) {
+                    const int row = r0 + 32 * (kb + k);
+                    const bool ok = tl.x0 + row < p.Wo;
+                    gu[k] = ok ? ldg16<true>(p.dz + ((pix0 + row) * 64 + ch * 8) * 2) : make_uint4(0, 0, 0, 0);
+                    xu[k] = ok ? ldg16<true>(p.xo + ((pix0 + row) * 64 + ch * 8) * 2) : make_uint4(0, 0, 0, 0);
                 }
-                *reinterpret_cast<uint4*>(sD + row * 128 + (((uint32_t)ch * 16u) ^ swz128(row))) = out;
+#pragma unroll
+                for (int k = 0; k < 2; ++k) {
+                    const int row = r0 + 32 * (kb + k);
+                    uint4 out = make_uint4(0, 0, 0, 0);
+                    if (tl.x0 + row < p.Wo) {
+                        float g[8], xv[8];
+                        unpack16<T>(gu[k], g);
+                        unpack16<T>(xu[k], xv);
+#pragma unroll
+                        for (int e = 0; e < 8; ++e) g[e] = cA[e] * g[e] - cB[e] * xv[e] + cC[e];
+                        out = pack16<T>(g);
+                    }
+                    *reinterpret_cast<uint4*>(sD + row * 128 + (((uint32_t)ch * 16u) ^ swz128(row))) = out;
+                }
+            }
+        } else {
+            const int oy_lo = tl.oy >> 1, oy_hi = min(pp.Hq - 1, (tl.oy + 1) >> 1);
+            const int selfy0 = (tl.oy - (oy_lo * 2 - 1)) * 3;
+            const long prow0 = ((long)tl.n * pp.Hq + oy_lo) * pp.Wq;
+#pragma unroll
+            for (int kb = 0; kb < 2; ++kb) {
+                const int row = 2 * r0 + 64 * kb;
+                const int ix = tl.x0 + row, j = ix >> 1;
+                const bool ok0 = ix < p.Wo, ok1 = ix + 1 < p.Wo;
+                uint4 xu[2], du[2][2];
+                uint2 au[2][2];
+                bool has[2][2];
+                xu[0] = ok0 ? ldg16<true>(p.xo + ((pix0 + row) * 64 + ch * 8) * 2) : make_uint4(0, 0, 0, 0);
+                xu[1] = ok1 ? ldg16<true>(p.xo + ((pix0 + row + 1) * 64 + ch * 8) * 2) : make_uint4(0, 0, 0, 0);
+#pragma unroll
+                for (int a = 0; a < 2; ++a)
+#pragma unroll
+                    for (int b = 0; b < 2; ++b) {
+                        has[a][b] = ok0 && oy_lo + a <= oy_hi && j + b <= pp.Wq - 1 && (b == 0 || ok1);
+                        au[a][b] = make_uint2(0xffffffffu, 0xffffffffu);
+                        du[a][b] = make_uint4(0, 0, 0, 0);
+                        if (has[a][b]) {
+                            const long o = (prow0 + (long)a * pp.Wq + j + b) * 64 + ch * 8;
+                            au[a][b] = *reinterpret_cast<const uint2*>(pp.argmax + o);
+                            du[a][b] = *reinterpret_cast<const uint4*>(pp.dyp + o * 2);
+                        }
+                    }
+#pragma unroll
+                for (int k = 0; k < 2; ++k) {
+                    uint4 out = make_uint4(0, 0, 0, 0);
+                    if (k == 0 ? ok0 : ok1) {
+                        float g[8], xv[8];
+                        unpack16<T>(xu[k], xv);
+#pragma unroll
+                        for (int e = 0; e < 8; ++e) g[e] = 0.f;
+#pragma unroll
+                        for (int w = 0; w < 4; ++w) {
+                            const int a = w >> 1, b = w & 1;
+                            if (b > k || !has[a][b]) continue;
+                            const int self = selfy0 - 6 * a + (b ? 0 : 1 + k);
+                            float d[8];
+                            unpack16<T>(du[a][b], d);
+                            const unsigned aw[2] = {au[a][b].x, au[a][b].y};
+#pragma unroll
+                            for (int e = 0; e < 8; ++e)
+                                if ((int)((aw[e >> 2] >> (8 * (e & 3))) & 0xff) == self) g[e] += d[e];
+                        }
+                        float sc[8], sh[8];
+#pragma unroll
+                        for (int e = 0; e < 8; e += 4) {
+                            *reinterpret_cast<float4*>(sc + e) = *reinterpret_cast<const float4*>(&sCoef[3][ch * 8 + e]);
+                            *reinterpret_cast<float4*>(sh + e) = *reinterpret_cast<const float4*>(&sCoef[4][ch * 8 + e]);
+                        }
+#pragma unroll
+                        for (int e = 0; e < 8; ++e) g[e] = (xv[e] * sc[e] + sh[e] > ElemTraits<T>::kReluBit) ? g[e] : 0.f;
+                        unpack16<T>(pack16<T>(g), g);
+#pragma unroll
+                        for (int e = 0; e < 8; ++e) g[e] = cA[e] * g[e] - cB[e] * xv[e] + cC[e];
+                        out = pack16<T>(g);
+                    }
+                    *reinterpret_cast<uint4*>(sD + (row + k) * 128 + (((uint32_t)ch * 16u) ^ swz128(row + k))) = out;
+                }
             }
         }
     };
@@ -1162,9 +1235,13 @@
 extern "C" int sm3_stem_wgrad_bn16(int dtype, const void* ximg, const void* dz, const void* xo, const float* mean,
                                    const float* invstd, const float* gamma, const double* global_sums, double count,
                                    const double* local_sums, float* dgamma, float* dbeta, float* dw, float* dw_slabs,
-                                   int N, int H, int W, int views, void* stream) {
-    if (!ximg || !dz || !xo || !mean || !invstd || !global_sums || !dw || count <= 0 || views < 1 || N % views)
+                                   int N, int H, int W, int views, void* stream, const uint8_t* argmax, const void* dy,
+                                   const float* scale, const float* shift) {
+    if (!ximg || !xo || !mean || !invstd || !global_sums || !dw || count <= 0 || views < 1 || N % views)
         return SM3_EINVAL;
+    const bool routed = !dz;
+    if (routed && (!argmax || !dy || !scale || !shift)) return SM3_EINVAL;
+    if (routed && (((uintptr_t)argmax & 7) || ((uintptr_t)dy & 15))) return SM3_EALIGN;
     if (dtype != SM3_BF16 && dtype != SM3_F16) return SM3_EDTYPE;
     if (dw_slabs && (((uintptr_t)dw_slabs | (uintptr_t)dw) & 15)) return SM3_EALIGN;
     StemWgrad16Params pp;
@@ -1180,11 +1257,17 @@
     p.mean = mean; p.invstd = invstd; p.gamma = gamma; p.gsums = global_sums; p.lsums = local_sums;
     p.dgamma = dgamma; p.dbeta = dbeta; p.dw = dw; p.dw_slabs = dw_slabs; p.inv_count = 1.0 / count;
     p.N = N; p.H = H; p.W = W; p.n_per_view = N / views; p.views = views;
+    pp.argmax = routed ? argmax : nullptr; pp.dyp = routed ? (const char*)dy : nullptr;
+    pp.scale = routed ? scale : nullptr; pp.shift = routed ? shift : nullptr;
+    pp.Hq = (p.Ho - 1) / 2 + 1; pp.Wq = (p.Wo - 1) / 2 + 1;
     const unsigned grid = (unsigned)(p.tiles < SM3_STEM_WGRAD_SLABS ? p.tiles : SM3_STEM_WGRAD_SLABS);
-    if (dtype == SM3_BF16)
-        hipLaunchKernelGGL(stem_wgrad16_kernel<bf16_t>, dim3(grid), dim3(256), 0, (hipStream_t)stream, pp);
-    else
-        hipLaunchKernelGGL(stem_wgrad16_kernel<f16_t>, dim3(grid), dim3(256), 0, (hipStream_t)stream, pp);
+    if (dtype == SM3_BF16) {
+        if (routed) hipLaunchKernelGGL((stem_wgrad16_kernel<bf16_t, true>), dim3(grid), dim3(256), 0, (hipStream_t)stream, pp);
+        else hipLaunchKernelGGL((stem_wgrad16_kernel<bf16_t, false>), dim3(grid), dim3(256), 0, (hipStream_t)stream, pp);
+    } else {
+        if (routed) hipLaunchKernelGGL((stem_wgrad16_kernel<f16_t, true>), dim3(grid), dim3(256), 0, (hipStream_t)stream, pp);
+        else hipLaunchKernelGGL((stem_wgrad16_kernel<f16_t, false>), dim3(grid), dim3(256), 0, (hipStream_t)stream, pp);
+    }
     SM3_CHECK_LAUNCH();
     return dw_slabs ? sm3_slab_reduce(dw_slabs, (int)grid, 64 * 147, dw, 1, stream) : 0;
 }
diff --git a/skin-sm3_amd/sm3hip/_lib.py b/skin-sm3_amd/sm3hip/_lib.py
--- a/skin-sm3_amd/sm3hip/_lib.py
+++ b/skin-sm3_amd/sm3hip/_lib.py
@@ -106,7 +106,7 @@
     "sm3_stem_image_cols": [_I],
     "sm3_stem_image_prep": [_I, _P, _P, _P, _I, _I, _I, _I, _P],
     "sm3_stem_conv_fwd16": [_I, _P, _P, _P, _P, _I, _I, _I, _P],
-    "sm3_stem_wgrad_bn16": [_I, _P, _P, _P, _P, _P, _P, _P, _D, _P, _P, _P, _P, _P, _I, _I, _I, _I, _P],
+    "sm3_stem_wgrad_bn16": [_I, _P, _P, _P, _P, _P, _P, _P, _D, _P, _P, _P, _P, _P, _I, _I, _I, _I, _P, _P, _P, _P, _P],
     "sm3_stem_dgrad_bn": [_I, _P, _P, _P, _P, _P, _P, _D, _P, _P, _I, _I, _I, _I, _P],
     "sm3_maxpool3x3s2_fwd": [_I, _P, _P, _P, _I, _I, _I, _I, _P],
     "sm3_maxpool3x3s2_bwd": [_I, _P, _P, _P, _I, _I, _I, _I, _P],
diff --git a/skin-sm3_amd/sm3hip/engine.py b/skin-sm3_amd/sm3hip/engine.py
--- a/skin-sm3_amd/sm3hip/engine.py
+++ b/skin-sm3_amd/sm3hip/engine.py
@@ -877,7 +877,9 @@
             taps["g"][0] = dcur.clone()
         Ho, Wo = ctx.stem_hw
         rs = ctx.stem
-        dz = torch.empty(N * Ho * Wo, 64, dtype=self.tdt, device=dfeat.device)
+        wg16 = isinstance(rs.x_in, ops.StemImage)
+        routed = wg16 and not self._data_only and dx_out is None
+        dz = None if routed else torch.empty(N * Ho * Wo, 64, dtype=self.tdt, device=dfeat.device)
         prow = ops.maxpool_bn_bwd_partial_rows(N, Ho, Wo, rs.V)
         part = self._work("fz_partials", rs.V * prow * 2 * 64)
         ops.maxpool_bn_bwd(self.dtype, ctx.argmax, dcur, rs.xo, rs.scale, rs.shift, rs.mean, rs.invstd, dz, part,
@@ -886,10 +888,11 @@
         gamma = self._bn_affine(rs.bu)[0]
         if not self._data_only:
             dgamma, dbeta = self._bn_affine(rs.bu, grad=True)
-            wg = ops.stem_wgrad_bn16 if isinstance(rs.x_in, ops.StemImage) else ops.stem_wgrad_bn
+            wg = ops.stem_wgrad_bn16 if wg16 else ops.stem_wgrad_bn
+            extra = {"routed": (ctx.argmax, dcur, rs.scale, rs.shift)} if routed else {}
             wg(self.dtype, rs.x_in, dz, rs.xo, rs.mean, rs.invstd, gamma, gsums, count, lsums, dgamma, dbeta,
                self._g(rs.cu.name + ".weight"), views=rs.V,
-               slabs=self._work("stem_slabs", ops.STEM_WGRAD_SLABS * 64 * 147) if self.det_wgrad else None)
+               slabs=self._work("stem_slabs", ops.STEM_WGRAD_SLABS * 64 * 147) if self.det_wgrad else None, **extra)
         if dx_out is not None:
             ops.stem_dgrad_bn(self.dtype, dz, rs.xo, rs.mean, rs.invstd, gamma, gsums, count,
                               self._p(rs.cu.name + ".weight"), dx_out, views=rs.V)
diff --git a/skin-sm3_amd/sm3hip/ops.py b/skin-sm3_amd/sm3hip/ops.py
--- a/skin-sm3_amd/sm3hip/ops.py
+++ b/skin-sm3_amd/sm3hip/ops.py
@@ -964,12 +964,12 @@
         if t.numel() < views * Cn:
             raise ValueError("maxpool_bn_bwd: per-channel vector too small")
     Ho, Wo = (H - 1) // 2 + 1, (W - 1) // 2 + 1
-    if x.numel() != N * H * W * Cn or dz.numel() != x.numel() or dy.numel() != N * Ho * Wo * Cn or \
+    if x.numel() != N * H * W * Cn or (dz is not None and dz.numel() != x.numel()) or dy.numel() != N * Ho * Wo * Cn or \
             argmax.numel() != dy.numel() or N % views:
         raise ValueError("maxpool_bn_bwd: size mismatch")
     if partials.numel() < views * maxpool_bn_bwd_partial_rows(N, H, W, views) * 2 * Cn:
         raise ValueError("maxpool_bn_bwd: partials too small")
-    with _prof("maxpool_bn_bwd", 0.0, _sz(dtype) * (2 * x.numel() + dy.numel()) + argmax.numel()):
+    with _prof("maxpool_bn_bwd", 0.0, _sz(dtype) * ((1 if dz is None else 2) * x.numel() + dy.numel()) + argmax.numel()):
         check(_lib.load().sm3_maxpool_bn_bwd(dtype, _ptr(argmax), _ptr(dy), _ptr(x), _ptr(scale), _ptr(shift), _ptr(mean),
                                              _ptr(invstd), _ptr(dz), _ptr(partials), N, H, W, Cn, views, _stream()),
               "sm3_maxpool_bn_bwd")
@@ -1097,27 +1097,43 @@
               "sm3_stem_conv_fwd16")
 
 
-def stem_wgrad_bn16(dtype, img, dz, xo, mean, invstd, gamma, gsums, count, lsums, dgamma, dbeta, dw, views=1, slabs=None):
-    tdt = TORCH_DTYPE[dtype]
+def stem_wgrad_bn16(dtype, img, dz, xo, mean, invstd, gamma, gsums, count, lsums, dgamma, dbeta, dw, views=1, slabs=None,
+                    routed=None):
+    tdt = TORCH_DTYPE[dtype]
+    if (dz is None) == (routed is None):
+        raise ValueError("stem_wgrad_bn16: exactly one of dz and routed=(argmax, dy, scale, shift)")
+    argmax, dy, scale, shift = routed if routed is not None else (None,) * 4
+    if routed is not None and any(t is None for t in routed):
+        raise ValueError("stem_wgrad_bn16: routed needs argmax, dy, scale and shift")
+    _chk(argmax, torch.uint8, "argmax"); _chk(dy, tdt, "dy"); _chk(scale, torch.float32, "scale"); _chk(shift, torch.float32, "shift")
     _chk(img.t, tdt, "ximg"); _chk(dz, tdt, "dz"); _chk(xo, tdt, "xo"); _chk(dw, torch.float32, "dw")
     for t in (mean, invstd, gamma, dgamma, dbeta):
         _chk(t, torch.float32)
     _chk(gsums, torch.float64); _chk(lsums, torch.float64); _chk(slabs, torch.float32, "slabs")
     N, Cc, H, W = img.shape
     Ho, Wo = (H - 1) // 2 + 1, (W - 1) // 2 + 1
-    if Cc != 3 or dz.numel() != N * Ho * Wo * 64 or xo.numel() != dz.numel() or dw.numel() < 64 * 147 or N % views or \
-            img.t.numel() != N * 3 * H * stem_image_cols(W):
+    if Cc != 3 or xo.numel() != N * Ho * Wo * 64 or (dz is not None and dz.numel() != xo.numel()) or \
+            dw.numel() < 64 * 147 or N % views or img.t.numel() != N * 3 * H * stem_image_cols(W):
         raise ValueError("stem_wgrad_bn16: size mismatch")
+    nbytes = _sz(dtype) * (img.t.numel() + 2 * xo.numel())
+    if routed is not None:
+        Hq, Wq = (Ho - 1) // 2 + 1, (Wo - 1) // 2 + 1
+        if dy.numel() != N * Hq * Wq * 64 or argmax.numel() != dy.numel():
+            raise ValueError("stem_wgrad_bn16: routed operand size mismatch")
+        if scale.numel() < views * 64 or shift.numel() < views * 64:
+            raise ValueError("stem_wgrad_bn16: scale/shift too small")
+        nbytes = _sz(dtype) * (img.t.numel() + xo.numel() + dy.numel()) + argmax.numel()
     if mean.numel() < views * 64 or invstd.numel() < views * 64 or gsums.numel() < views * 128 or \
             (lsums is not None and lsums.numel() < views * 128):
         raise ValueError("stem_wgrad_bn16: per-channel vector too small")
     if slabs is not None and slabs.numel() < STEM_WGRAD_SLABS * 64 * 147:
         raise ValueError("stem_wgrad_bn16: slab workspace too small")
     M = N * Ho * Wo
-    with _prof("stem_wgrad_bn", 2.0 * M * 64 * 147, _sz(dtype) * (img.t.numel() + 2 * dz.numel())):
+    with _prof("stem_wgrad_bn", 2.0 * M * 64 * 147, nbytes):
         check(_lib.load().sm3_stem_wgrad_bn16(dtype, _ptr(img.t), _ptr(dz), _ptr(xo), _ptr(mean), _ptr(invstd), _ptr(gamma),
                                               _ptr(gsums), float(count), _ptr(lsums), _ptr(dgamma), _ptr(dbeta), _ptr(dw),
-                                              _ptr(slabs), N, H, W, views, _stream()), "sm3_stem_wgrad_bn16")
+                                              _ptr(slabs), N, H, W, views, _stream(), _ptr(argmax), _ptr(dy), _ptr(scale),
+                                              _ptr(shift)), "sm3_stem_wgrad_bn16")
 
 
 def stem_dgrad_bn(dtype, dz, xo, mean, invstd, gamma, gsums, count, w_master, dx, views=1):
```

New measurement: 4595. About the same (-0.3%).
